# andrewcharlesjones/spatial-alignment

Measured on AMD Instinct MI355X. Metric: training steps/sec (ELBO fwd+bwd), 2-view N=10k M=200, 1/2/4/8 GPU, higher is better.
Workload: dtype f32 (fp64 warp layer, covariance whitening and M x M factorisations)

## Files before the change

include/gpsa_hip.h:

```cpp
#ifndef GPSA_HIP_H
#define GPSA_HIP_H

#ifdef __cplusplus
extern "C" {
#endif

enum {
  GPSA_F32 = 0,
  GPSA_F64 = 1,
  GPSA_F32_X64 = 2,
  GPSA_F32_OUT64 = 3,
  GPSA_F32_ACC64 = 4
};
enum { GPSA_K_RBF = 0, GPSA_K_MATERN12 = 1, GPSA_K_MATERN32 = 2 };
enum { GPSA_EINVAL = -1, GPSA_EWORKSPACE = -2, GPSA_EUNSUPPORTED = -3 };

int gpsa_version(void);
const char* gpsa_build_arch(void);
const char* gpsa_source_hash(void);

int gpsa_kmat(int dtype, int in_dtype, int kind, const void* Z, int M, const void* X, long long C,
              int D, const void* ls_u, const void* var_u, double jitter, void* K, void* stream);

long long gpsa_kmat_bwd_workspace(int dtype, int M, long long C, int D);
// ... 93 lines not shown
                                     long long workspace_bytes, void* stream);

long long gpsa_whiten_workspace(int M);
int gpsa_whiten_f64(const double* Kinv, int in_dtype, const void* Kuf, int M, long long C,
                    int alpha_dtype, void* alpha, double* q, void* workspace, long long workspace_bytes,
                    void* stream);

int gpsa_panel_mm(int dtype, int p_dtype, int transP, const void* P, const void* X, int M, long long C,
                  void* Y, void* colsq, void* workspace, long long workspace_bytes, void* stream);

int gpsa_col_axpy(int dtype, const void* Y, const void* X, const void* d, double s, int M,
                  long long C, void* out, void* stream);

int gpsa_data_sample_fwd(const float* meanT, const float* v, const double* q, const float* var_u,
                         const float* eps, long long C, int L, float* F, float* Sigma, void* stream);
int gpsa_data_sample_bwd(const float* dF, const float* eps, const float* Sigma, const float* var_u,
                         long long C, int L, float* g, float* dmeanT, float* qbar, int dvar_dtype, void* dvar_u,
                         void* workspace, long long workspace_bytes, void* stream);
int gpsa_warp_sample_fwd(const double* meanT, const double* v, const double* q, const float* var_u,
                         const float* X, const float* slopes, const float* intercept,
                         const float* eps, long long n, int D, int S, float* Gmean, float* Gs,
                         double* Gs64, int* bad, void* stream);
int gpsa_warp_sample_bwd(const float* dGmean, const float* dGs, const double* dGs64, const float* eps,
                         const float* var_u, const float* X, long long n, int D, int S, double* dmeanT, double* g,
                         double* qbar, float* dvar_u, float* dslopes, float* dintercept,
                         void* workspace, long long workspace_bytes, void* stream);

int gpsa_mean_resid_fwd(const float* Z, const float* slopes, const float* intercept,
                        const float* delta, int M, int D, double scale, float* mu_z, double* resid,
                        void* stream);
int gpsa_mean_resid_bwd(const double* dresid, const float* Z, const float* slopes, int M, int D,
                        double scale, float* ddelta, float* dZ, float* dslopes, float* dintercept,
                        void* stream);

int gpsa_loglik_fwd(const float* F, const float* Y, const float* noise_u, int S, long long N, int P,
                    double* out, void* workspace, long long workspace_bytes, void* stream);
int gpsa_loglik_bwd(const float* F, const float* Y, const float* noise_u, const double* gout, int S,
                    long long N, int P, float* dF, float* dnoise_u, void* workspace,
                    long long workspace_bytes, void* stream);

int gpsa_bdot(int dtype, const void* A, long long strideA, const void* B, long long strideB,
              long long n, int batch, void* out, void* workspace, long long workspace_bytes,
              void* stream);
int gpsa_add_diag(int dtype, void* A, int M, int batch, double s, void* stream);

int gpsa_mvn_kl_fwd(const double* Kinv, const double* logdetK, const double* Omega,
                    long long omega_stride, const double* logdetO, long long logdet_stride,
                    const double* Dm, const double* KD, int M, int L, double* kl, void* stream);
int gpsa_mvn_kl_bwd(const double* Kuu, const double* Kinv, const double* Omega, long long omega_stride,
                    const double* Oinv, long long oinv_stride, const double* Dm, const double* KD,
                    const double* g, int M, int L, double* dOmega, double* dDm, double* Sp,
                    void* stream);

int gpsa_mvn_kl_grouped_fwd(const double* mats, const double* inv, const double* logdet,
                            const int* om_idx, const int* pr_idx, const double* D, int M, int T,
                            double* kl, double* KD, void* stream);
int gpsa_mvn_kl_grouped_bwd(const double* mats, const double* inv, const int* om_idx,
                            const int* pr_list, const int* grp_off, const int* order, const double* D,
                            const double* KD, const double* g, int M, int T, int P, double* dOmega,
                            double* dD, double* S, void* stream);

int gpsa_elbo_fwd(const double* ll, int n_ll, const double* kl, int n_kl, double kl_scale, float* loss,
                  void* stream);
int gpsa_elbo_bwd(const float* gloss, int n_ll, int n_kl, double kl_scale, double* dll, double* dkl,
                  void* stream);

long long gpsa_kmeans_workspace(long long N, int D, int K);
int gpsa_kmeans_assign(const float* X, long long N, int D, const float* centres, int K, int* assign,
                       float* d2, void* stream);
int gpsa_kmeans_update(const float* X, const int* assign, long long N, int D, int K, float* centres,
                       int* counts, void* workspace, long long workspace_bytes, void* stream);


int gpsa_kmat_batched(int kind, const float* Z, long long strideZ, int M, const float* X, long long strideX,
                      long long C, int D, const float* ls_u, const float* var_u, int stride_par,
                      const long long* n_live, int batch, double jitter, double* K, long long strideK,
                      void* stream);
long long gpsa_kmat_bwd_batched_workspace(int M, long long C, int D, int batch);
int gpsa_kmat_bwd_batched(int kind, const float* Z, long long strideZ, int M, const float* X, long long strideX,
                          long long C, int D, const float* ls_u, const float* var_u, int stride_par,
                          const long long* n_live, int batch, const double* Kbar, long long strideK, int same,
                          double* dZ, long long stride_dZ, double* dparams, void* workspace,
                          long long workspace_bytes, void* stream);
int gpsa_kmat_bwd_x64(int kind, const float* Z, int M, const double* X, long long C, int D, const float* ls_u,
                      const float* var_u, const float* Kbar, double* dZ, double* dX, double* dparams,
                      void* workspace, long long workspace_bytes, void* stream);
int gpsa_kmat_bwd_x64_f64(int kind, const float* Z, int M, const double* X, long long C, int D, const float* ls_u,
                          const float* var_u, const double* Kbar, double* dZ, double* dX, double* dparams,
                          void* workspace, long long workspace_bytes, void* stream);
int gpsa_kmat_bwd_x64_f64_axpy(int kind, const float* Z, int M, const double* X, long long C, int D, const float* ls_u,
                               const float* var_u, const double* Kbar, const double* X2, const float* d, double s,
                               double* dZ, double* dX, double* dparams, void* workspace, long long workspace_bytes,
                               void* stream);
long long gpsa_exact_dkuu_workspace(int M, long long C);
int gpsa_exact_dkuu_f64(const double* G, const double* A, const float* d, int M, long long C, double* dK,
                        void* workspace, long long workspace_bytes, void* stream);
long long gpsa_longk_f64_workspace(int M, long long K, int nprob);
int gpsa_longk_f64(int nprob, const double* const* G, const double* const* B, const void* const* d, int d_dtype,
                   int M, long long K, long long ld, int sym, const double* alpha, const double* beta,
                   double* const* out, void* workspace, long long workspace_bytes, void* stream);
int gpsa_kmat_bwd_x64_axpy(int kind, const float* Z, int M, const double* X, long long C, int D, const float* ls_u,
                           const float* var_u, const float* Kbar, const float* X2, const float* d, double s,
                           double* dZ, double* dX, double* dparams, void* workspace, long long workspace_bytes,
                           void* stream);
int gpsa_whiten_f64_dual(const double* Kinv, const double* Kuf, int M, long long C, double* alpha64, float* alpha32,
                         double* q, void* workspace, long long workspace_bytes, void* stream);

int gpsa_whiten_gen_f64_dual(const double* Kinv, int kind, const float* Z, const double* X64, int D, const float* ls_u,
                             const float* var_u, int M, long long C, double* alpha64, float* alpha32, double* q,
                             void* workspace, long long workspace_bytes, void* stream);
int gpsa_whiten_axpy_f32(const double* Kinv, const float* X, int M, long long C, const float* X2, const float* d,
                         double s, float* out, void* workspace, long long workspace_bytes, void* stream);
int gpsa_whiten_batched_f64(const double* Kinv, long long strideKinv, const double* Kuf, int M, long long C,
                            long long strideX, double* alpha, double* q, int batch, void* workspace,
                            long long workspace_bytes, void* stream);
int gpsa_quadform_fwd_keep_batched_f64(const double* alpha, const double* Omega, int M, long long C, int L,
                                       double* v, double* W, const double* dcT, double* meanT, int batch,
                                       void* stream);
int gpsa_quadform_bwd_alpha_kept_batched_f64(const double* W, const double* g, int M, long long C, int L,
                                             const double* dcT, const double* dmeanT, double* dalpha,
                                             int batch, void* stream);
int gpsa_col_axpy_batched_f64(const double* Y, const double* X, const double* d, double s, int M, long long C,
                              double* out, int batch, void* stream);
long long gpsa_gram_batched_workspace(int M, long long C, int L, int batch);
int gpsa_gram_batched_f64(const double* alpha, const double* g, int M, long long C, int L, double* dOmega,
                          int batch, void* workspace, long long workspace_bytes, void* stream);
int gpsa_mvn_kl_grouped_bwd_acc(const double* mats, const double* inv, const int* om_idx,
                                const int* pr_list, const int* grp_off, const int* order, const double* D,
                                const double* KD, const double* g, int M, int T, int P, double* dOmega,
                                double* dD, double* S, int accumulate, void* stream);

#define GPSA_MAX_MODS 4

typedef struct gpsa_step_desc {
  int n_views, n_dims, n_mods, n_samples;
  int m_x, m_g;
  int kind_warp, kind_data;
  int n_latent[GPSA_MAX_MODS];
  int n_out[GPSA_MAX_MODS];
  int has_lmc[GPSA_MAX_MODS];
  long long n_rows[GPSA_MAX_MODS];
  int s_test;
  long long n_test[GPSA_MAX_MODS];
  int want_kl;
  const int* view_fixed;
  const long long* view_rows;
  long long keep_budget_bytes;
  int exact_inducing_grad;
  int kl_own_lo, kl_own_hi;
  int contraction;
} gpsa_step_desc;

typedef struct gpsa_step_params {
  const float* Xtilde;
  const float* delta_G;
  const float* Omega_sqt_G;
  const float* warp_ls;
  const float* warp_var;
  const float* slopes;
  const float* intercepts;
  const float* Gtilde;
  const float* data_ls;
  const float* data_var;
  const float* Omega_sqt_F[GPSA_MAX_MODS];
  const float* delta_F[GPSA_MAX_MODS];
  const float* W[GPSA_MAX_MODS];
} gpsa_step_params;

typedef struct gpsa_step_param_grads {
  float *Xtilde, *delta_G, *Omega_sqt_G, *warp_ls, *warp_var, *Gtilde, *data_ls, *data_var;
  float* Omega_sqt_F[GPSA_MAX_MODS];
  float* delta_F[GPSA_MAX_MODS];
  float* W[GPSA_MAX_MODS];
} gpsa_step_param_grads;

typedef struct gpsa_step_io {
  const float* X[GPSA_MAX_MODS];
  const float* eps_G;
  const float* eps_F[GPSA_MAX_MODS];
  const float* G_test[GPSA_MAX_MODS];
  const float* eps_F_test[GPSA_MAX_MODS];
  float* G_means[GPSA_MAX_MODS];
  float* G_samples[GPSA_MAX_MODS];
  float* F_latent[GPSA_MAX_MODS];
  float* F_obs[GPSA_MAX_MODS];
  float* F_latent_test[GPSA_MAX_MODS];
  float* F_obs_test[GPSA_MAX_MODS];
  float* mu_z;
  double* kl;
  int* flag;
  int keep_products;
  int reuse_mm;
  int fuse_elbo;
  const float* Y[GPSA_MAX_MODS];
  const float* noise_u[GPSA_MAX_MODS];
  double* ll_part[GPSA_MAX_MODS];
  float* F_fused_T[GPSA_MAX_MODS];
  double* bwd_acc;
  int bwd_acc_mode;
  void* f_event;
  const float* loss_src;
  float* loss_dst;
  int skip_missing;
} gpsa_step_io;

typedef struct gpsa_step_out_grads {
  const float* dG_means[GPSA_MAX_MODS];
  const float* dG_samples[GPSA_MAX_MODS];
  const float* dF_latent[GPSA_MAX_MODS];
  const float* dF_obs[GPSA_MAX_MODS];
  const float* dF_latent_test[GPSA_MAX_MODS];
  const float* dF_obs_test[GPSA_MAX_MODS];
  const double* dkl;
// ... 139 lines not shown
```

spatial_alignment_amd/_lib.py:

```python
import ctypes as C
import os

_HERE = os.path.dirname(os.path.abspath(__file__))
LIB_PATH = os.path.join(_HERE, "libgpsa_hip.so")

_vp, _i, _ll, _d = C.c_void_p, C.c_int, C.c_longlong, C.c_double

SIGNATURES = {
    "gpsa_version": (_i, []),
    "gpsa_build_arch": (C.c_char_p, []),
    "gpsa_source_hash": (C.c_char_p, []),
    "gpsa_kmat": (_i, [_i, _i, _i, _vp, _i, _vp, _ll, _i, _vp, _vp, _d, _vp, _vp]),
    "gpsa_kmat_bwd_workspace": (_ll, [_i, _i, _ll, _i]),
    "gpsa_kmat_bwd": (_i, [_i, _i, _i, _vp, _i, _vp, _ll, _i, _vp, _vp, _vp, _i, _vp, _vp, _vp, _vp, _ll, _vp]),
    "gpsa_gemm_workspace": (_ll, [_i, _i, _i, _i, _i]),
    "gpsa_gemm": (_i, [_i, _i, _i, _i, _i, _ll, _d, _vp, _ll, _ll, _vp, _ll, _ll, _d, _vp, _ll, _ll,
                       _i, _i, _vp, _ll, _vp]),
    "gpsa_omega_fwd": (_i, [_vp, _i, _i, _d, _vp, _vp]),
    "gpsa_omega_bwd": (_i, [_vp, _vp, _i, _i, _i, _vp, _vp]),
    "gpsa_omega_fwd2": (_i, [_vp, _i, _vp, _vp, _i, _vp, _i, _d, _vp]),
    "gpsa_omega_bwd2": (_i, [_vp, _vp, _vp, _i, _vp, _vp, _vp, _i, _i, _i, _vp]),
    "gpsa_chol_f64": (_i, [_vp, _i, _i, _vp, _vp, _vp]),
    "gpsa_tri_inv_f64": (_i, [_vp, _vp, _i, _i, _vp]),
    "gpsa_chol_inv_f64": (_i, [_vp, _vp, _i, _i, _vp, _vp, _vp]),
# ... 15 lines not shown
    "gpsa_quadform_bwd_omega_delta_x3": (_i, [_i, _vp, _vp, _vp, _i, _ll, _i, _vp, _vp, _d, _vp, _ll, _vp]),
    "gpsa_whiten_workspace": (_ll, [_i]),
    "gpsa_whiten_f64": (_i, [_vp, _i, _vp, _i, _ll, _i, _vp, _vp, _vp, _ll, _vp]),
    "gpsa_panel_mm": (_i, [_i, _i, _i, _vp, _vp, _i, _ll, _vp, _vp, _vp, _ll, _vp]),
    "gpsa_col_axpy": (_i, [_i, _vp, _vp, _vp, _d, _i, _ll, _vp, _vp]),
    "gpsa_data_sample_fwd": (_i, [_vp, _vp, _vp, _vp, _vp, _ll, _i, _vp, _vp, _vp]),
    "gpsa_data_sample_bwd": (_i, [_vp, _vp, _vp, _vp, _ll, _i, _vp, _vp, _vp, _i, _vp, _vp, _ll, _vp]),
    "gpsa_warp_sample_fwd": (_i, [_vp, _vp, _vp, _vp, _vp, _vp, _vp, _vp, _ll, _i, _i, _vp, _vp, _vp, _vp, _vp]),
    "gpsa_warp_sample_bwd": (_i, [_vp, _vp, _vp, _vp, _vp, _vp, _ll, _i, _i, _vp, _vp, _vp, _vp, _vp, _vp, _vp,
                                  _ll, _vp]),
    "gpsa_mean_resid_fwd": (_i, [_vp, _vp, _vp, _vp, _i, _i, _d, _vp, _vp, _vp]),
    "gpsa_mean_resid_bwd": (_i, [_vp, _vp, _vp, _i, _i, _d, _vp, _vp, _vp, _vp, _vp]),
    "gpsa_loglik_fwd": (_i, [_vp, _vp, _vp, _i, _ll, _i, _vp, _vp, _ll, _vp]),
    "gpsa_loglik_bwd": (_i, [_vp, _vp, _vp, _vp, _i, _ll, _i, _vp, _vp, _vp, _ll, _vp]),
    "gpsa_bdot": (_i, [_i, _vp, _ll, _vp, _ll, _ll, _i, _vp, _vp, _ll, _vp]),
    "gpsa_add_diag": (_i, [_i, _vp, _i, _i, _d, _vp]),
    "gpsa_mvn_kl_fwd": (_i, [_vp, _vp, _vp, _ll, _vp, _ll, _vp, _vp, _i, _i, _vp, _vp]),
    "gpsa_mvn_kl_bwd": (_i, [_vp, _vp, _vp, _ll, _vp, _ll, _vp, _vp, _vp, _i, _i, _vp, _vp, _vp, _vp]),
    "gpsa_mvn_kl_grouped_fwd": (_i, [_vp, _vp, _vp, _vp, _vp, _vp, _i, _i, _vp, _vp, _vp]),
    "gpsa_mvn_kl_grouped_bwd": (_i, [_vp, _vp, _vp, _vp, _vp, _vp, _vp, _vp, _vp, _i, _i, _i, _vp, _vp, _vp,
                                     _vp]),
    "gpsa_elbo_fwd": (_i, [_vp, _i, _vp, _i, _d, _vp, _vp]),
    "gpsa_elbo_bwd": (_i, [_vp, _i, _i, _d, _vp, _vp, _vp]),
    "gpsa_kmeans_workspace": (_ll, [_ll, _i, _i]),
    "gpsa_kmeans_assign": (_i, [_vp, _ll, _i, _vp, _i, _vp, _vp, _vp]),
    "gpsa_kmeans_update": (_i, [_vp, _vp, _ll, _i, _i, _vp, _vp, _vp, _ll, _vp]),
}

MAX_MODS = 4


class StepDesc(C.Structure):
    _fields_ = [
        ("n_views", _i), ("n_dims", _i), ("n_mods", _i), ("n_samples", _i),
        ("m_x", _i), ("m_g", _i), ("kind_warp", _i), ("kind_data", _i),
        ("n_latent", _i * MAX_MODS), ("n_out", _i * MAX_MODS), ("has_lmc", _i * MAX_MODS),
        ("n_rows", _ll * MAX_MODS), ("s_test", _i), ("n_test", _ll * MAX_MODS), ("want_kl", _i),
        ("view_fixed", C.POINTER(_i)), ("view_rows", C.POINTER(_ll)), ("keep_budget_bytes", _ll),
        ("exact_inducing_grad", _i), ("kl_own_lo", _i), ("kl_own_hi", _i), ("contraction", _i),
    ]


class StepParams(C.Structure):
    _fields_ = [
        ("Xtilde", _vp), ("delta_G", _vp), ("Omega_sqt_G", _vp), ("warp_ls", _vp), ("warp_var", _vp),
        ("slopes", _vp), ("intercepts", _vp), ("Gtilde", _vp), ("data_ls", _vp), ("data_var", _vp),
        ("Omega_sqt_F", _vp * MAX_MODS), ("delta_F", _vp * MAX_MODS), ("W", _vp * MAX_MODS),
    ]


class StepParamGrads(C.Structure):
    _fields_ = [
        ("Xtilde", _vp), ("delta_G", _vp), ("Omega_sqt_G", _vp), ("warp_ls", _vp), ("warp_var", _vp),
        ("Gtilde", _vp), ("data_ls", _vp), ("data_var", _vp),
        ("Omega_sqt_F", _vp * MAX_MODS), ("delta_F", _vp * MAX_MODS), ("W", _vp * MAX_MODS),
    ]


class StepIO(C.Structure):
    _fields_ = [
        ("X", _vp * MAX_MODS), ("eps_G", _vp), ("eps_F", _vp * MAX_MODS), ("G_test", _vp * MAX_MODS),
        ("eps_F_test", _vp * MAX_MODS), ("G_means", _vp * MAX_MODS), ("G_samples", _vp * MAX_MODS),
        ("F_latent", _vp * MAX_MODS), ("F_obs", _vp * MAX_MODS), ("F_latent_test", _vp * MAX_MODS),
        ("F_obs_test", _vp * MAX_MODS), ("mu_z", _vp), ("kl", _vp), ("flag", _vp), ("keep_products", _i),
        ("reuse_mm", _i), ("fuse_elbo", _i), ("Y", _vp * MAX_MODS), ("noise_u", _vp * MAX_MODS),
        ("ll_part", _vp * MAX_MODS), ("F_fused_T", _vp * MAX_MODS), ("bwd_acc", _vp), ("bwd_acc_mode", _i),
        ("f_event", _vp), ("loss_src", _vp), ("loss_dst", _vp), ("skip_missing", _i),
    ]


class StepOutGrads(C.Structure):
    _fields_ = [
        ("dG_means", _vp * MAX_MODS), ("dG_samples", _vp * MAX_MODS), ("dF_latent", _vp * MAX_MODS),
        ("dF_obs", _vp * MAX_MODS), ("dF_latent_test", _vp * MAX_MODS), ("dF_obs_test", _vp * MAX_MODS),
        ("dkl", _vp), ("gloss", _vp),
    ]


_pp = C.POINTER(_vp)

SIGNATURES.update({
    "gpsa_kmat_batched": (_i, [_i, _vp, _ll, _i, _vp, _ll, _ll, _i, _vp, _vp, _i, C.POINTER(_ll), _i, _d, _vp, _ll, _vp]),
    "gpsa_kmat_bwd_batched_workspace": (_ll, [_i, _ll, _i, _i]),
    "gpsa_kmat_bwd_batched": (_i, [_i, _vp, _ll, _i, _vp, _ll, _ll, _i, _vp, _vp, _i, C.POINTER(_ll), _i, _vp, _ll, _i,
                                   _vp, _ll, _vp, _vp, _ll, _vp]),
    "gpsa_kmat_bwd_x64": (_i, [_i, _vp, _i, _vp, _ll, _i, _vp, _vp, _vp, _vp, _vp, _vp, _vp, _ll, _vp]),
    "gpsa_kmat_bwd_x64_f64": (_i, [_i, _vp, _i, _vp, _ll, _i, _vp, _vp, _vp, _vp, _vp, _vp, _vp, _ll, _vp]),
    "gpsa_kmat_bwd_x64_f64_axpy": (_i, [_i, _vp, _i, _vp, _ll, _i, _vp, _vp, _vp, _vp, _vp, _d, _vp, _vp, _vp, _vp, _ll,
                                        _vp]),
    "gpsa_exact_dkuu_workspace": (_ll, [_i, _ll]),
    "gpsa_exact_dkuu_f64": (_i, [_vp, _vp, _vp, _i, _ll, _vp, _vp, _ll, _vp]),
    "gpsa_longk_f64_workspace": (_ll, [_i, _ll, _i]),
    "gpsa_longk_f64": (_i, [_i, _vp, _vp, _vp, _i, _i, _ll, _ll, _i, _vp, _vp, _vp, _vp, _ll, _vp]),
    "gpsa_kmat_bwd_x64_axpy": (_i, [_i, _vp, _i, _vp, _ll, _i, _vp, _vp, _vp, _vp, _vp, _d, _vp, _vp, _vp, _vp, _ll,
                                    _vp]),
    "gpsa_thin_update_f32": (_i, [_vp, _i, _i, _vp, _ll, _vp, _vp]),
    "gpsa_whiten_f64_dual": (_i, [_vp, _vp, _i, _ll, _vp, _vp, _vp, _vp, _ll, _vp]),
    "gpsa_whiten_gen_f64_dual": (_i, [_vp, _i, _vp, _vp, _i, _vp, _vp, _i, _ll, _vp, _vp, _vp, _vp, _ll, _vp]),
    "gpsa_whiten_axpy_f32": (_i, [_vp, _vp, _i, _ll, _vp, _vp, _d, _vp, _vp, _ll, _vp]),
    "gpsa_whiten_batched_f64": (_i, [_vp, _ll, _vp, _i, _ll, _ll, _vp, _vp, _i, _vp, _ll, _vp]),
    "gpsa_quadform_fwd_keep_batched_f64": (_i, [_vp, _vp, _i, _ll, _i, _vp, _vp, _vp, _vp, _i, _vp]),
    "gpsa_quadform_bwd_alpha_kept_batched_f64": (_i, [_vp, _vp, _i, _ll, _i, _vp, _vp, _vp, _i, _vp]),
    "gpsa_col_axpy_batched_f64": (_i, [_vp, _vp, _vp, _d, _i, _ll, _vp, _i, _vp]),
    "gpsa_gram_batched_workspace": (_ll, [_i, _ll, _i, _i]),
    "gpsa_gram_batched_f64": (_i, [_vp, _vp, _i, _ll, _i, _vp, _i, _vp, _ll, _vp]),
    "gpsa_mvn_kl_grouped_bwd_acc": (_i, [_vp, _vp, _vp, _vp, _vp, _vp, _vp, _vp, _vp, _i, _i, _i, _vp, _vp, _vp, _i,
                                         _vp]),
    "gpsa_step_create": (_vp, [C.POINTER(StepDesc)]),
    "gpsa_step_describe": (_i, [C.POINTER(StepDesc), C.POINTER(_ll)]),
    "gpsa_step_destroy": (None, [_vp]),
    "gpsa_step_saved_bytes": (_ll, [_vp]),
    "gpsa_step_saved_bytes_nokeep": (_ll, [_vp]),
    "gpsa_quadform_keep_f32_workspace": (_ll, [_i, _i]),
    "gpsa_quadform_fwd_keep_f32": (_i, [_i, _vp, _vp, _i, _ll, _i, _vp, _vp, _vp, _ll, _vp]),
    "gpsa_quadform_keep_f32_bytes": (_ll, [_i, _ll, _i]),
    "gpsa_quadform_bwd_alpha_kept_f32": (_i, [_vp, _vp, _i, _ll, _i, _vp, _vp, _vp, _vp]),
    "gpsa_lmc_loglik_workspace": (_ll, [_ll, _i, _i, _i]),
    "gpsa_lmc_loglik_fused_f32": (_i, [_vp, _vp, _vp, _vp, _i, _ll, _i, _i, _vp, _i, _vp, _vp, _vp, _ll, _vp]),
    "gpsa_quadform_elbo_parts": (_i, []),
    "gpsa_quadform_elbo_f32_workspace": (_ll, [_i, _ll, _i]),
    "gpsa_quadform_elbo_f32": (_i, [_i, _vp, _vp, _i, _ll, _i, _vp, _vp, _vp, _vp, _vp, _ll, _i, _vp, _vp, _vp, _vp, _vp,
                                    _vp, _vp, _ll, _vp]),
    "gpsa_quadform_elbo_takes_delta": (_i, [_i]),
    "gpsa_quadform_elbo_x3_f32_workspace": (_ll, [_i, _ll, _i]),
    "gpsa_quadform_elbo_x3_f32": (_i, [_i, _vp, _vp, _i, _ll, _i, _vp, _vp, _vp, _vp, _vp, _ll, _i, _vp, _vp, _vp, _vp,
                                       _vp, _vp, _vp, _ll, _vp]),
    "gpsa_quadform_elbo_delta_x3_f32": (_i, [_i, _vp, _vp, _i, _ll, _i, _vp, _vp, _vp, _vp, _vp, _ll, _i, _vp, _vp, _vp,
                                             _vp, _vp, _vp, _vp, _ll, _vp]),
    "gpsa_quadform_elbo_delta_f32": (_i, [_i, _vp, _vp, _i, _ll, _i, _vp, _vp, _vp, _vp, _vp, _ll, _i, _vp, _vp, _vp, _vp,
                                          _vp, _vp, _vp, _ll, _vp]),
    "gpsa_step_scratch_bytes": (_ll, [_vp]),
    "gpsa_step_bwd_acc_bytes": (_ll, [_vp]),
    "gpsa_step_n_kl": (_i, [_vp]),
    "gpsa_step_n_factorised": (_i, [_vp]),
    "gpsa_step_eps_g_numel": (_ll, [_vp]),
    "gpsa_step_batch_layout": (_i, [_vp, C.POINTER(_ll)]),
    "gpsa_step_graph": (_i, [_vp, _i, C.POINTER(_ll)]),
    "gpsa_step_early_backwards": (_ll, [_vp]),
    "gpsa_stream_capture_id": (C.c_ulonglong, [_vp]),
    "gpsa_step_timing": (_i, [_vp, _i]),
    "gpsa_step_timing_read": (_i, [_vp, _vp, _i]),
    "gpsa_step_forward": (_i, [_vp, C.POINTER(StepParams), C.POINTER(StepIO), _vp, _vp, _i, _vp]),
    "gpsa_step_backward": (_i, [_vp, C.POINTER(StepParams), C.POINTER(StepIO), C.POINTER(StepOutGrads), _vp, _vp,
                                C.POINTER(StepParamGrads), _vp]),
    "gpsa_elbo_loss_fwd": (_i, [_i, _pp, _pp, _pp, C.POINTER(_i), C.POINTER(_ll), C.POINTER(_i), _vp, _i, _d, _vp,
                                _vp, _vp, _ll, _vp]),
    "gpsa_elbo_loss_bwd": (_i, [_i, _pp, _pp, _pp, C.POINTER(_i), C.POINTER(_ll), C.POINTER(_i), _vp, _i, _d, _pp, _pp,
                                _vp, _i, _vp, _vp, _ll, _vp]),
    "gpsa_elbo_loss_fused_fwd": (_i, [_i, _pp, _pp, _pp, C.POINTER(_i), C.POINTER(_ll), C.POINTER(_i), _pp, _i, _vp, _i,
                                      _d, _vp, _vp, _vp, _ll, _vp]),
    "gpsa_elbo_loss_fused_bwd": (_i, [_i, _pp, _pp, _pp, C.POINTER(_i), C.POINTER(_ll), C.POINTER(_i), _pp, _i, _vp, _i,
                                      _d, _pp, _pp, _vp, _i, _vp, _vp, _ll, _vp]),
    "gpsa_elbo_fused_post": (_i, [_vp, _vp, _vp, _i, _ll, _i, _vp, _vp, _i, _vp, _vp, _ll, _vp]),
    "gpsa_step_fused": (_i, [_vp, _i]),
    "gpsa_step_contraction": (_i, [_vp, _i]),
    "gpsa_adam_step": (_i, [_i, _pp, _pp, _pp, _pp, C.POINTER(_ll), _d, _d, _d, _d, _vp, _vp]),
    "gpsa_row_sample_gather": (_i, [_i, C.POINTER(_i), C.POINTER(_ll), C.POINTER(_ll), C.c_ulonglong, _vp, _pp,
                                    C.POINTER(_i), _pp, C.POINTER(_i), _pp, _pp, _pp, _vp]),
    "gpsa_elbo_loss_weighted_fwd": (_i, [_i, _pp, _pp, _pp, C.POINTER(_i), C.POINTER(_ll), C.POINTER(_i),
                                         C.POINTER(_i), _pp, _pp, _vp, _i, _d, _vp, _vp, _vp, _ll, _vp]),
    "gpsa_elbo_loss_weighted_bwd": (_i, [_i, _pp, _pp, _pp, C.POINTER(_i), C.POINTER(_ll), C.POINTER(_i),
                                         C.POINTER(_i), _pp, _pp, _vp, _i, _d, _pp, _pp, _vp, _i, _vp, _vp, _ll, _vp]),
    "gpsa_quadform_elbo_skip_f32": (_i, [_i, _vp, _vp, _i, _ll, _i, _vp, _vp, _vp, _vp, _vp, _ll, _i, _vp, _vp, _vp, _vp,
                                         _vp, _vp, _vp, _ll, _vp]),
    "gpsa_quadform_elbo_delta_skip_f32": (_i, [_i, _vp, _vp, _i, _ll, _i, _vp, _vp, _vp, _vp, _vp, _ll, _i, _vp, _vp, _vp,
                                               _vp, _vp, _vp, _vp, _ll, _vp]),
    "gpsa_count_observed_workspace": (_ll, []),
    "gpsa_count_observed": (_i, [_i, _pp, C.POINTER(_ll), C.POINTER(_i), C.POINTER(_i), _pp, _pp, _vp, _ll, _vp]),
    "gpsa_elbo_loss_skip_fwd": (_i, [_i, _pp, _pp, _pp, C.POINTER(_i), C.POINTER(_ll), C.POINTER(_i), _pp, _i,
                                     C.POINTER(_i), _pp, _pp, _pp, _vp, _i, _d, _vp, _vp, _vp, _ll, _vp]),
    "gpsa_elbo_loss_skip_bwd": (_i, [_i, _pp, _pp, _pp, C.POINTER(_i), C.POINTER(_ll), C.POINTER(_i), _pp, _i,
                                     C.POINTER(_i), _pp, _pp, _pp, _vp, _i, _d, _pp, _pp, _vp, _i, _vp, _vp, _ll, _vp]),
    "gpsa_lmc_loglik_fused_skip_f32": (_i, [_vp, _vp, _vp, _vp, _i, _ll, _i, _i, _vp, _i, _vp, _vp, _vp, _ll, _vp]),
    "gpsa_predict_moments_f32": (_i, [_vp, _vp, _vp, _vp, _ll, _i, _i, _i, _vp, _vp, _i, _vp, _vp, _vp, _vp, _vp, _vp,
                                      _vp]),
    "gpsa_predict_counts_f32": (_i, [_vp, _vp, _vp, _vp, _ll, _i, _i, _i, _vp, _vp, _vp, _vp, _vp, _vp, _vp]),
    "gpsa_lgamma_sum_workspace": (_ll, []),
    "gpsa_lgamma_sum": (_i, [_i, _pp, C.POINTER(_ll), C.POINTER(_i), C.POINTER(_i), _pp, _i, _pp, _vp, _ll, _vp]),
    "gpsa_elbo_loss_pois_fwd": (_i, [_i, _pp, _pp, _pp, C.POINTER(_i), C.POINTER(_ll), C.POINTER(_i), _pp, _i,
                                     C.POINTER(_i), _pp, _pp, _pp, C.POINTER(_i), _pp, _pp, _i, _vp, _i, _d, _vp, _vp,
                                     _vp, _ll, _vp]),
    "gpsa_elbo_loss_pois_bwd": (_i, [_i, _pp, _pp, _pp, C.POINTER(_i), C.POINTER(_ll), C.POINTER(_i), _pp, _i,
                                     C.POINTER(_i), _pp, _pp, _pp, C.POINTER(_i), _pp, _pp, _i, _vp, _i, _d, _pp, _pp,
                                     _vp, _i, _vp, _vp, _ll, _vp]),
    "gpsa_quadform_elbo_pois_f32": (_i, [_i, _vp, _vp, _i, _ll, _i, _vp, _vp, _vp, _vp, _vp, _ll, _i, _vp, _vp, _vp, _vp,
                                         _vp, _vp, _vp, _i, _vp, _ll, _vp]),
    "gpsa_quadform_elbo_delta_pois_f32": (_i, [_i, _vp, _vp, _i, _ll, _i, _vp, _vp, _vp, _vp, _vp, _ll, _i, _vp, _vp, _vp,
                                               _vp, _vp, _vp, _vp, _i, _vp, _ll, _vp]),
    "gpsa_lmc_loglik_fused_pois_f32": (_i, [_vp, _vp, _vp, _vp, _i, _i, _ll, _i, _i, _vp, _i, _vp, _vp, _vp, _ll, _vp]),
    "gpsa_step_likelihood": (_i, [_vp, _i, _i, _vp]),
# ... 73 lines not shown
```

spatial_alignment_amd/csrc/internal.hpp:

```cpp
#pragma once
#include "common.hpp"

namespace gpsa {

template <typename T>
int gemm_launch(int transA, int transB, int m, int n, long long k, double alpha, const T* A, long long lda,
                long long sA, const T* B, long long ldb, long long sB, double beta, T* C, long long ldc,
                long long sC, int batch, int splitk, void* ws, long long ws_bytes, hipStream_t st);
enum { GEMM_TRI_NONE = 0, GEMM_TRI_UPPER_A = 1, GEMM_TRI_LOWER_C = 2, GEMM_TRI_LTL = 3 };
template <typename T>
int gemm_launch_tri(int transA, int transB, int m, int n, long long k, double alpha, const T* A, long long lda,
                    long long sA, const T* B, long long ldb, long long sB, double beta, T* C, long long ldc,
                    long long sC, int batch, int splitk, void* ws, long long ws_bytes, hipStream_t st, int tri);
template <typename TIA, typename TIB, typename TO>
int gemm64_launch(int transA, int transB, int m, int n, long long k, double alpha, const TIA* A, long long lda,
                  long long sA, const TIB* B, long long ldb, long long sB, double beta, TO* C, long long ldc,
                  long long sC, int batch, int splitk, void* ws, long long ws_bytes, hipStream_t st);

int omega_fwd_dma_launch(const float* A0, int n0, double* O0, const float* A1, int n1, double* O1, int M, double jitter,
                         hipStream_t st);

int omega_bwd_dma_launch(const double* G0, const float* A0, float* D0, int n0, const double* G1, const float* A1,
                         float* D1, int n1, int M, hipStream_t st);

int mvn_kl_grouped_fwd_slices(int M);
int mvn_kl_grouped_fwd_copy(const double* mats, const double* inv, const double* logdet, const int* om_idx,
                            const int* pr_idx, const double* D, int M, int T, double* kl, double* KD,
                            double* kl_copy, double* part, int* cnt, hipStream_t st);

int lmc_mfma_launch(const float* F, const float* W, const float* Y, const float* noise_u, int S, long long N, int L,
                    int P, double* zpart, int nparts, float* dF, float* dWpart, int G, hipStream_t st);
int lmc_mfma_skip_launch(const float* F, const float* W, const float* Y, const float* noise_u, int S, long long N, int L,
                         int P, double* zpart, int nparts, float* dF, float* dWpart, int G, hipStream_t st);

constexpr int LOSS_MAX_VIEWS = 64;
struct ViewRows {
  long long off[LOSS_MAX_VIEWS + 1];
};
static inline bool views_ok(int V, const long long* off, long long N) {
  if (V < 1 || V > LOSS_MAX_VIEWS || off == nullptr || off[0] != 0 || off[V] != N) return false;
  for (int v = 0; v < V; ++v)
    if (off[v + 1] < off[v]) return false;
  return true;
}
static inline ViewRows view_rows(long long N, int V, const long long* off) {
  ViewRows vr;
  if (off != nullptr) {
    for (int v = 0; v <= V; ++v) vr.off[v] = off[v];
  } else {
    vr.off[0] = 0;
    vr.off[1] = N;
  }
  return vr;
}

int pois_loglik_launch(bool bwd, const float* F, const float* Y, const float* log_offset, int S, long long N, int P,
                       const ViewRows& vr, int V, int nb, const double* w, const float* gloss, int skip, float* dF,
                       double* part, hipStream_t st);
int lmc_mfma_pois_launch(const float* F, const float* W, const float* Y, const float* log_offset, int skip, int S,
                         long long N, int L, int P, double* zpart, int nparts, float* dF, float* dWpart, int G,
                         hipStream_t st);

bool proj64_ok(int MB, long long C, int batch);
template <typename TI>
int proj64_launch(int MB, const double* Apk, const TI* X, int M, long long C, double* alpha, float* out32, double* q,
                  int batch, long long sX, hipStream_t st, bool q_zeroed);
int zero_fill_async(void* ptr, size_t bytes, hipStream_t st);
int copy_async(void* dst, const void* src, size_t bytes, hipStream_t st);
int elbo_fused_post_ticket(float* g_ext, float* dmeanT, float* abar, int M, long long C, int L, const float* gloss,
                           const float* var_u, double* dvar_u, double* part, int* tick, hipStream_t st);
int proj64_gen_launch(int MB, const double* Apk, int kind, const float* Z, const double* X64, int D, const float* ls_u,
                      const float* var_u, int M, long long C, double* alpha, float* out32, double* q, hipStream_t st,
                      bool q_zeroed);

}
```

spatial_alignment_amd/csrc/kl.hip:

```cpp
#include "common.hpp"

namespace gpsa {

__global__ void __launch_bounds__(1024)
mvn_kl_fwd_kernel(const double* __restrict__ Kinv, const double* __restrict__ logdetK,
                  const double* __restrict__ Omega, long long omega_stride,
                  const double* __restrict__ logdetO, long long logdet_stride,
                  const double* __restrict__ Dm, const double* __restrict__ KD, int M, int L,
                  double* __restrict__ kl) {
  __shared__ double red[16];
  const int l = blockIdx.x;
  const double* Om = Omega + (long long)l * omega_stride;
  double acc = 0.0;
  for (int e = threadIdx.x; e < M * M; e += 1024) acc += Kinv[e] * Om[e];
  for (int m = threadIdx.x; m < M; m += 1024) acc += KD[(long long)m * L + l] * Dm[(long long)m * L + l];
  const double t = block_sum(acc, red);
  if (threadIdx.x == 0)
    kl[l] = 0.5 * (logdetK[0] - logdetO[(long long)l * logdet_stride] + t - (double)M);
}

__global__ void __launch_bounds__(256)
mvn_kl_bwd_kernel(const double* __restrict__ Kuu, const double* __restrict__ Kinv,
                  const double* __restrict__ Omega, long long omega_stride,
                  const double* __restrict__ Oinv, long long oinv_stride,
// ... 23 lines not shown
                          const int* __restrict__ pr_idx, const double* __restrict__ D, int M,
                          double* __restrict__ kl, double* __restrict__ KD, double* __restrict__ kl_copy,
                          double* part, int* cnt) {
  __shared__ double red[16];
  const int t = blockIdx.x, lane = threadIdx.x & 63, w = threadIdx.x >> 6;
  const int q = blockIdx.y, NS = gridDim.y;
  const int p = pr_idx[t], o = om_idx[t];
  if (p < 0) {
    if (q != 0) return;
    if (threadIdx.x == 0) {
      kl[t] = 0.0;
      if (kl_copy != nullptr) kl_copy[t] = 0.0;
    }
    for (int m = threadIdx.x; m < M; m += 1024) KD[(long long)t * M + m] = 0.0;
    return;
  }
  const double* Ki = inv + (long long)p * M * M;
  const double* Om = mats + (long long)o * M * M;
  const double* d = D + (long long)t * M;
  double acc = 0.0;
  for (int i0 = w + 64 * q; i0 < M; i0 += 64 * NS) {
    double tr[4] = {0.0, 0.0, 0.0, 0.0}, kd[4] = {0.0, 0.0, 0.0, 0.0};
    for (int j0 = 0; j0 < M; j0 += 256) {
      double kv[4][4], ov[4][4], dv[4];
#pragma unroll
      for (int q = 0; q < 4; ++q) {
        const int j = j0 + lane + 64 * q;
        dv[q] = j < M ? d[j < M ? j : M - 1] : 0.0;
#pragma unroll
        for (int r = 0; r < 4; ++r) {
          const int i = i0 + 16 * r;
          const long long e = (long long)(i < M ? i : M - 1) * M + (j < M ? j : M - 1);
          kv[r][q] = Ki[e];
          ov[r][q] = Om[e];
        }
      }
#pragma unroll
      for (int r = 0; r < 4; ++r)
#pragma unroll
        for (int q = 0; q < 4; ++q) {
          const bool ok = i0 + 16 * r < M && j0 + lane + 64 * q < M;
          const double k = ok ? kv[r][q] : 0.0;
          tr[r] += k * ov[r][q];
          kd[r] += k * dv[q];
        }
    }
#pragma unroll
    for (int r = 0; r < 4; ++r) {
      const int i = i0 + 16 * r;
      if (i < M) {
        const double s = wave_sum(kd[r]);
        if (lane == 0) {
          KD[(long long)t * M + i] = s;
          acc += s * d[i];
        }
        acc += tr[r];
      }
    }
  }
  double tot = block_sum(acc, red);
  if (threadIdx.x == 0) {
    if (NS > 1) {
      part[(long long)t * NS + q] = tot;
      __threadfence();
      if (atomicAdd(&cnt[t], 1) != NS - 1) return;
      __threadfence();
      tot = 0.0;
      for (int i = 0; i < NS; ++i) tot += __hip_atomic_load(&part[(long long)t * NS + i], __ATOMIC_RELAXED, __HIP_MEMORY_SCOPE_AGENT);
      cnt[t] = 0;
    }
    const double v = 0.5 * (logdet[p] - logdet[o] + tot - (double)M);
    kl[t] = v;
    if (kl_copy != nullptr) kl_copy[t] = v;
  }
}

__global__ void __launch_bounds__(256)
mvn_kl_grouped_bwd_kernel(const double* __restrict__ mats, const double* __restrict__ inv,
                          const int* __restrict__ om_idx,
                          const int* __restrict__ pr_list, const int* __restrict__ grp_off,
                          const int* __restrict__ order, const double* __restrict__ D,
                          const double* __restrict__ KD, const double* __restrict__ g, int M, int T, int P,
                          double* __restrict__ dOmega, double* __restrict__ dD, double* __restrict__ S,
                          int accumulate) {
  const long long mm = (long long)M * M, e = blockIdx.x * 256LL + threadIdx.x;
  const int pg = blockIdx.y;
  const int t0 = grp_off[pg], t1 = grp_off[pg + 1];
  if (pg == P) {
    if (blockIdx.x == 0)
      for (int q = t0; q < t1; ++q)
        for (int m = threadIdx.x; m < M; m += 256) dD[(long long)order[q] * M + m] = 0.0;
    if (!accumulate && e < mm)
      for (int q = t0; q < t1; ++q) dOmega[(long long)order[q] * mm + e] = 0.0;
    return;
  }
  const int p = pr_list[pg];
  if (blockIdx.x == 0)
    for (int q = t0; q < t1; ++q) {
      const int t = order[q];
      for (int m = threadIdx.x; m < M; m += 256) dD[(long long)t * M + m] = g[t] * KD[(long long)t * M + m];
    }
  if (e >= mm) return;
  const int i = (int)(e / M), j = (int)(e % M);
  const double kinv = inv[(long long)p * mm + e];
  double s0 = 0.0, s1 = 0.0, gs = 0.0;
  for (int q = t0; q < t1; q += 8) {
    double ga[8], om[8], oi[8], di[8], dj[8], old[8];
    int tt[8];
#pragma unroll
    for (int u = 0; u < 8; ++u) {
      const bool on = q + u < t1;
      const int ta = order[on ? q + u : t0];
      tt[u] = on ? ta : -1;
      ga[u] = on ? g[ta] : 0.0;
      const long long mo = (long long)om_idx[ta] * mm + e;
      om[u] = mats[mo];
      oi[u] = inv[mo];
      di[u] = D[(long long)ta * M + i];
      dj[u] = D[(long long)ta * M + j];
      old[u] = (accumulate && on) ? dOmega[(long long)ta * mm + e] : 0.0;
    }
#pragma unroll
    for (int u = 0; u < 8; ++u)
      if (tt[u] >= 0) dOmega[(long long)tt[u] * mm + e] = old[u] + 0.5 * ga[u] * (kinv - oi[u]);
#pragma unroll
    for (int u = 0; u < 8; u += 2) {
      gs += ga[u] + ga[u + 1];
      s0 += ga[u] * (om[u] + di[u] * dj[u]);
      s1 += ga[u + 1] * (om[u + 1] + di[u + 1] * dj[u + 1]);
    }
  }
  S[(long long)pg * mm + e] = gs * mats[(long long)p * mm + e] - (s0 + s1);
}

int mvn_kl_grouped_fwd_slices(int M) { return M > 64 ? (M + 63) / 64 < 8 ? (M + 63) / 64 : 8 : 1; }
int mvn_kl_grouped_fwd_copy(const double* mats, const double* inv, const double* logdet, const int* om_idx,
                            const int* pr_idx, const double* D, int M, int T, double* kl, double* KD,
                            double* kl_copy, double* part, int* cnt, hipStream_t st) {
  if (M < 1 || T < 1) return GPSA_EINVAL;
  const int ns = (part != nullptr && cnt != nullptr) ? mvn_kl_grouped_fwd_slices(M) : 1;
  mvn_kl_grouped_fwd_kernel<<<dim3((unsigned)T, (unsigned)ns), 1024, 0, st>>>(mats, inv, logdet, om_idx, pr_idx, D, M, kl,
                                                                             KD, kl_copy, part, cnt);
  GPSA_LAUNCH_CHECK();
  return 0;
}

}

extern "C" {

int gpsa_mvn_kl_grouped_fwd(const double* mats, const double* inv, const double* logdet,
                            const int* om_idx, const int* pr_idx, const double* D, int M, int T,
                            double* kl, double* KD, void* stream) {
  if (M < 1 || T < 1) return GPSA_EINVAL;
  gpsa::mvn_kl_grouped_fwd_kernel<<<T, 1024, 0, as_stream(stream)>>>(mats, inv, logdet, om_idx, pr_idx, D,
                                                                     M, kl, KD, nullptr, nullptr, nullptr);
  GPSA_LAUNCH_CHECK();
  return 0;
}

int gpsa_mvn_kl_grouped_bwd_acc(const double* mats, const double* inv, const int* om_idx,
                                const int* pr_list, const int* grp_off, const int* order, const double* D,
                                const double* KD, const double* g, int M, int T, int P, double* dOmega,
                                double* dD, double* S, int accumulate, void* stream) {
  if (M < 1 || T < 1 || P < 1) return GPSA_EINVAL;
  dim3 grid((unsigned)cdiv((long long)M * M, 256), (unsigned)(P + 1));
  gpsa::mvn_kl_grouped_bwd_kernel<<<grid, 256, 0, as_stream(stream)>>>(
      mats, inv, om_idx, pr_list, grp_off, order, D, KD, g, M, T, P, dOmega, dD, S, accumulate);
  GPSA_LAUNCH_CHECK();
  return 0;
}

int gpsa_mvn_kl_grouped_bwd(const double* mats, const double* inv, const int* om_idx,
                            const int* pr_list, const int* grp_off, const int* order, const double* D,
                            const double* KD, const double* g, int M, int T, int P, double* dOmega,
                            double* dD, double* S, void* stream) {
  return gpsa_mvn_kl_grouped_bwd_acc(mats, inv, om_idx, pr_list, grp_off, order, D, KD, g, M, T, P, dOmega,
                                     dD, S, 0, stream);
}

int gpsa_mvn_kl_fwd(const double* Kinv, const double* logdetK, const double* Omega,
                    long long omega_stride, const double* logdetO, long long logdet_stride,
                    const double* Dm, const double* KD, int M, int L, double* kl, void* stream) {
  if (M < 1 || L < 1) return GPSA_EINVAL;
  gpsa::mvn_kl_fwd_kernel<<<L, 1024, 0, as_stream(stream)>>>(Kinv, logdetK, Omega, omega_stride, logdetO,
                                                             logdet_stride, Dm, KD, M, L, kl);
  GPSA_LAUNCH_CHECK();
  return 0;
}

int gpsa_mvn_kl_bwd(const double* Kuu, const double* Kinv, const double* Omega, long long omega_stride,
                    const double* Oinv, long long oinv_stride, const double* Dm, const double* KD,
                    const double* g, int M, int L, double* dOmega, double* dDm, double* Sp,
                    void* stream) {
  if (M < 1 || L < 1) return GPSA_EINVAL;
  const unsigned nb = (unsigned)cdiv((long long)M * M, 256);
  gpsa::mvn_kl_bwd_kernel<<<nb, 256, 0, as_stream(stream)>>>(Kuu, Kinv, Omega, omega_stride, Oinv,
                                                             oinv_stride, Dm, KD, g, M, L, dOmega, dDm, Sp);
  GPSA_LAUNCH_CHECK();
  return 0;
}

}
```

spatial_alignment_amd/csrc/kmat.hip:

```cpp
#include "common.hpp"
#include "kmat_cov.hpp"

namespace gpsa {

constexpr int KM_ROWS = 16;

constexpr int KM_MAXB = 16;
struct KmatBatch {
  long long sZ, sX, sK;
  int sP, ragged;
  long long n[KM_MAXB];
  const void* axX;
  const float* axd;
  float axs;
};
static inline KmatBatch kmat_single() {
  KmatBatch kb;
  kb.sZ = kb.sX = kb.sK = 0;
  kb.sP = kb.ragged = 0;
  kb.axX = nullptr;
  kb.axd = nullptr;
  kb.axs = 0.f;
  for (int i = 0; i < KM_MAXB; ++i) kb.n[i] = 0;
  return kb;
}

template <typename TI, typename TX, typename T, int KIND>
__global__ void __launch_bounds__(256)
kmat_fwd_kernel(const TI* __restrict__ Z, int M, const TX* __restrict__ X, long long C, int D,
                const TI* __restrict__ ls_u, const TI* __restrict__ var_u, T jitter,
                T* __restrict__ K, KmatBatch kb) {
  __shared__ T Zs[KM_ROWS][MAXD];
  const int b = blockIdx.z;
  Z += b * kb.sZ;
  X += b * kb.sX;
  K += b * kb.sK;
  ls_u += b * kb.sP;
  var_u += b * kb.sP;
  const long long live = kb.ragged ? kb.n[b] : C;
  const int m0 = blockIdx.y * KM_ROWS;
  if (threadIdx.x < KM_ROWS * MAXD) {
    int r = threadIdx.x / MAXD, d = threadIdx.x % MAXD;
    Zs[r][d] = (m0 + r < M && d < D) ? (T)Z[(long long)(m0 + r) * D + d] : T(0);
  }
  __syncthreads();
  const long long c = blockIdx.x * 256LL + threadIdx.x;
  if (c >= C) return;
  const int mend = min(KM_ROWS, M - m0);
  if (c >= live) {
    for (int r = 0; r < mend; ++r) K[(long long)(m0 + r) * C + c] = T(0);
    return;
  }
  const T ell = t_exp<T>((T)ls_u[0]), inv_ell = T(1) / ell, var = t_exp<T>((T)var_u[0]);
  T x[MAXD];
#pragma unroll
  for (int d = 0; d < MAXD; ++d) x[d] = (d < D) ? (T)X[c * D + d] : T(0);
  for (int r = 0; r < mend; ++r) {
    T k, cd, pl;
    cov_eval<T, KIND>(Zs[r], x, D, ell, inv_ell, var, k, cd, pl);
    if ((long long)(m0 + r) == c) k += jitter;
    K[(long long)(m0 + r) * C + c] = k;
  }
}

constexpr int KB_MCHUNK = 32;
constexpr int KB_MCHUNK_SMALL = 8;
static inline int kb_rows(int M, long long C) {
  return (cdiv(C, 256) * cdiv(M, KB_MCHUNK) < 1024) ? KB_MCHUNK_SMALL : KB_MCHUNK;
}
constexpr int KB_MAXBX = 1024;
constexpr int KB_D2_ROWS = 16;
static inline int kmat_bwd_d2_rows() { return KB_D2_ROWS; }
static inline bool kmat_bwd_d2(int M, long long Ctot, int D) {
  (void)M;
  (void)Ctot;
  return D == 2;
}

template <typename TI, typename T, int KIND, int MCH, typename TK = T, typename TX = TI>
__global__ void __launch_bounds__(256)
kmat_bwd_kernel(const TI* __restrict__ Z, int M, const TX* __restrict__ X, long long C, int D,
                const TI* __restrict__ ls_u, const TI* __restrict__ var_u,
                const TK* __restrict__ Kbar, T* __restrict__ zpart, T* __restrict__ xpart,
                T* __restrict__ spart, KmatBatch bt) {
  {
    const long long b = blockIdx.z;
    Z += b * bt.sZ;
    X += b * bt.sX;
    Kbar += b * bt.sK;
    ls_u += b * bt.sP;
    var_u += b * bt.sP;
    zpart += b * (long long)gridDim.x * M * D;
    if (xpart != nullptr) xpart += b * (long long)gridDim.y * C * D;
    spart += b * (long long)gridDim.x * gridDim.y * 2;
  }
  const long long nlive = bt.ragged ? bt.n[blockIdx.z] : C;
  __shared__ T Zs[MCH][MAXD];
  __shared__ T acc[4][MCH][MAXD];
  __shared__ T red[4];
  const int lane = threadIdx.x & 63, w = threadIdx.x >> 6;
  const int m0 = blockIdx.y * MCH;
  const int mc = min(MCH, M - m0);
  const T ell = t_exp<T>((T)ls_u[0]), inv_ell = T(1) / ell, var = t_exp<T>((T)var_u[0]);
  if (threadIdx.x < MCH * MAXD) {
    const int r = threadIdx.x / MAXD, d = threadIdx.x % MAXD;
    Zs[r][d] = (r < mc && d < D) ? (T)Z[(long long)(m0 + r) * D + d] : T(0);
  }
  for (int i = threadIdx.x; i < 4 * MCH * MAXD; i += 256) (&acc[0][0][0])[i] = T(0);
  __syncthreads();
  T s_ls = T(0), s_var = T(0);
  const long long ncb = (C + 255) / 256;
  for (long long cb = blockIdx.x; cb < ncb; cb += gridDim.x) {
    const long long c = cb * 256 + threadIdx.x;
    const bool live = c < nlive;
    T x[MAXD], dx[MAXD];
#pragma unroll
    for (int d = 0; d < MAXD; ++d) {
      x[d] = (live && d < D) ? (T)X[c * D + d] : T(0);
      dx[d] = T(0);
    }
    const T axc = (bt.axX != nullptr && live) ? (T)bt.axs * (T)bt.axd[c] : T(0);
    for (int r = 0; r < mc; ++r) {
      T k, cd, pl;
      cov_eval<T, KIND>(Zs[r], x, D, ell, inv_ell, var, k, cd, pl);
      T kb = live ? (T)Kbar[(long long)(m0 + r) * C + c] : T(0);
      if (bt.axX != nullptr && live)
        kb += axc * (T)reinterpret_cast<const TK*>(bt.axX)[(long long)(m0 + r) * C + c];
      s_ls += kb * pl;
      s_var += kb * k;
      T wgt = kb * cd;
#pragma unroll
      for (int d = 0; d < MAXD; ++d)
        if (d < D) {
          T t = wgt * (Zs[r][d] - x[d]);
          dx[d] -= t;
          T tz = wave_sum(t);
          if (lane == 0) acc[w][r][d] += tz;
        }
    }
    if (xpart != nullptr && c < C) {
      T* xr = xpart + (long long)blockIdx.y * C * D;
      for (int d = 0; d < D; ++d) xr[c * D + d] = dx[d];
    }
  }
  __syncthreads();
  T* zrow = zpart + (long long)blockIdx.x * M * D;
  for (int i = threadIdx.x; i < mc * D; i += 256) {
    const int r = i / D, d = i % D;
    zrow[(long long)(m0 + r) * D + d] = acc[0][r][d] + acc[1][r][d] + acc[2][r][d] + acc[3][r][d];
  }
  T* sp = spart + ((long long)blockIdx.x * gridDim.y + blockIdx.y) * 2;
  T a = block_sum(s_ls, red);
  if (threadIdx.x == 0) sp[0] = a;
  T b2 = block_sum(s_var, red);
  if (threadIdx.x == 0) sp[1] = b2;
}

template <typename TI, typename T, int KIND, int MCH, typename TK = T, typename TX = TI>
__global__ void __launch_bounds__(256, 2)
kmat_bwd_d2_kernel(const TI* __restrict__ Z, int M, int rows, const TX* __restrict__ X, long long C,
                   const TI* __restrict__ ls_u, const TI* __restrict__ var_u,
                   const TK* __restrict__ Kbar, T* __restrict__ zpart, T* __restrict__ xpart,
                   T* __restrict__ spart, KmatBatch bt) {
  constexpr int D = 2;
  static_assert(MCH % 8 == 0, "the closing reduction takes 8 rows at a time");
  {
    const long long b = blockIdx.z;
    Z += b * bt.sZ;
    X += b * bt.sX;
    Kbar += b * bt.sK;
    ls_u += b * bt.sP;
    var_u += b * bt.sP;
    zpart += b * (long long)gridDim.x * M * D;
    if (xpart != nullptr) xpart += b * (long long)gridDim.y * C * D;
    spart += b * (long long)gridDim.x * gridDim.y * 2;
  }
  const long long nlive = bt.ragged ? bt.n[blockIdx.z] : C;
  constexpr int RSTR = 256 + 16;
  __shared__ T Zs[MCH][MAXD];
  __shared__ T rbuf[16 * RSTR];
  __shared__ T red[4];
  const int m0 = blockIdx.y * rows;
  const int mc = min(rows, M - m0);
  const T ell = t_exp<T>((T)ls_u[0]), inv_ell = T(1) / ell, var = t_exp<T>((T)var_u[0]);
  if (threadIdx.x < MCH * MAXD) {
    const int r = threadIdx.x / MAXD, d = threadIdx.x % MAXD;
    Zs[r][d] = (r < mc && d < D) ? (T)Z[(long long)(m0 + r) * D + d] : T(0);
  }
  __syncthreads();
  T tz[MCH][D];
#pragma unroll
  for (int r = 0; r < MCH; ++r) tz[r][0] = tz[r][1] = T(0);
  T s_ls = T(0), s_var = T(0);
  const long long ncb = (C + 255) / 256;
  struct Col {
    long long c;
    bool live;
    T x0, x1, axc;
  };
  const bool two = bt.axX != nullptr;
  const TK* __restrict__ axp = reinterpret_cast<const TK*>(bt.axX);
  auto load = [&](long long cb, TK(&kraw)[MCH], TK(&araw)[MCH], Col& q) {
    q.c = cb * 256 + threadIdx.x;
    q.live = q.c < nlive;
    q.x0 = q.x1 = q.axc = T(0);
    const long long cc = q.live ? q.c : 0;
    if (q.live) {
      q.x0 = (T)X[q.c * D];
      q.x1 = (T)X[q.c * D + 1];
    }
    if (two) {
      if (q.live) q.axc = (T)bt.axs * (T)bt.axd[q.c];
#pragma unroll
      for (int r = 0; r < MCH; ++r) {
        const long long o = (long long)min(m0 + r, M - 1) * C + cc;
        kraw[r] = Kbar[o];
        araw[r] = axp[o];
      }
    } else {
#pragma unroll
      for (int r = 0; r < MCH; ++r) {
        kraw[r] = Kbar[(long long)min(m0 + r, M - 1) * C + cc];
        araw[r] = TK(0);
      }
    }
  };
  auto compute = [&](const TK(&kraw)[MCH], const TK(&araw)[MCH], const Col& q) {
    const T x[MAXD] = {q.x0, q.x1, T(0), T(0)};
    T dx0 = T(0), dx1 = T(0);
    int zo = 0;
    asm volatile("" : "+v"(zo));
    const T(*Zr)[MAXD] = Zs + zo;
#pragma unroll
    for (int r = 0; r < MCH; ++r) {
      T k, cd, pl;
      cov_eval<T, KIND>(Zr[r], x, D, ell, inv_ell, var, k, cd, pl);
      const T kb = (q.live && r < mc) ? (T)kraw[r] + q.axc * (T)araw[r] : T(0);
      s_ls += kb * pl;
      s_var += kb * k;
      const T wgt = kb * cd;
      const T t0 = wgt * (Zr[r][0] - x[0]), t1 = wgt * (Zr[r][1] - x[1]);
      dx0 -= t0;
      dx1 -= t1;
      tz[r][0] += t0;
      tz[r][1] += t1;
      if ((r & 3) == 3) __builtin_amdgcn_sched_barrier(0);
    }
    if (xpart != nullptr && q.c < C) {
      T* xr = xpart + (long long)blockIdx.y * C * D;
      xr[q.c * D] = dx0;
      xr[q.c * D + 1] = dx1;
    }
  };
  for (long long cb = blockIdx.x; cb < ncb; cb += gridDim.x) {
    TK k0[MCH];
    TK a0[MCH];
    Col q0;
    load(cb, k0, a0, q0);
    __builtin_amdgcn_sched_barrier(0);
    compute(k0, a0, q0);
  }
  T* zrow = zpart + (long long)blockIdx.x * M * D;
#pragma unroll
  for (int r0 = 0; r0 < MCH; r0 += 8) {
    __syncthreads();
#pragma unroll
    for (int q = 0; q < 8; ++q) {
      rbuf[(2 * q) * RSTR + threadIdx.x] = tz[r0 + q][0];
      rbuf[(2 * q + 1) * RSTR + threadIdx.x] = tz[r0 + q][1];
    }
    __syncthreads();
    const int v = threadIdx.x >> 4, sub = threadIdx.x & 15;
    T a = T(0);
#pragma unroll
    for (int i = 0; i < 16; ++i) a += rbuf[v * RSTR + sub + 16 * i];
    a += dpp_move<0xB1>(a);
    a += dpp_move<0x4E>(a);
    a += dpp_move<0x141>(a);
    a += dpp_move<0x140>(a);
    const int r = r0 + (v >> 1);
    if (sub == 0 && r < mc) zrow[(long long)(m0 + r) * D + (v & 1)] = a;
  }
  T* sp = spart + ((long long)blockIdx.x * gridDim.y + blockIdx.y) * 2;
  T a = block_sum(s_ls, red);
  if (threadIdx.x == 0) sp[0] = a;
  T b2 = block_sum(s_var, red);
  if (threadIdx.x == 0) sp[1] = b2;
}

template <typename T, typename TO>
__global__ void __launch_bounds__(256)
kmat_bwd_finish_kernel(const T* __restrict__ zpart, long long nbx, long long nz,
                       const T* __restrict__ xpart, long long nby, long long nx,
                       const T* __restrict__ spart, long long ns, int same, TO* __restrict__ dZ,
                       TO* __restrict__ dX, TO* __restrict__ dparams, long long sdZ, long long sdX) {
  {
    const long long b = blockIdx.y;
    zpart += b * nbx * nz;
    if (xpart != nullptr) xpart += b * nby * nx;
    spart += b * ns * 2;
    dZ += b * sdZ;
    if (dX != nullptr) dX += b * sdX;
    dparams += b * 2;
  }
  __shared__ double red[256];
  const long long zb = (nz + 15) / 16, xb = (nx + 63) / 64;
  const T* part;
  long long rows, stride, n, col;
  int ng, grp, sub;
  TO* dst;
  long long blk = blockIdx.x;
  bool fold = false;
  if (blk < zb) {
    ng = 16; grp = threadIdx.x >> 4; sub = threadIdx.x & 15;
    part = zpart; rows = nbx; stride = nz; n = nz; col = blk * 16 + sub; dst = dZ; fold = same != 0;
  } else if (blk < zb + xb) {
    blk -= zb;
    if (xpart == nullptr || dX == nullptr || same) return;
    ng = 4; grp = threadIdx.x >> 6; sub = threadIdx.x & 63;
    part = xpart; rows = nby; stride = nx; n = nx; col = blk * 64 + sub; dst = dX;
  } else {
    ng = 16; grp = threadIdx.x >> 4; sub = threadIdx.x & 15;
    part = spart; rows = ns; stride = 2; n = 2; col = sub; dst = dparams;
  }
  double a0 = 0.0, a1 = 0.0, a2 = 0.0, a3 = 0.0;
  if (col < n) {
    long long r = grp;
    for (; r + 3 * ng < rows; r += 4 * ng) {
      a0 += (double)part[r * stride + col];
      a1 += (double)part[(r + ng) * stride + col];
      a2 += (double)part[(r + 2 * ng) * stride + col];
      a3 += (double)part[(r + 3 * ng) * stride + col];
    }
    for (; r < rows; r += ng) a0 += (double)part[r * stride + col];
    if (fold)
      for (long long q = grp; q < nby; q += ng) a1 += (double)xpart[q * nx + col];
  }
  const int width = 256 / ng;
  red[grp * width + sub] = (a0 + a1) + (a2 + a3);
  __syncthreads();
  if (grp == 0 && col < n) {
    double t = 0.0;
    for (int q = 0; q < ng; ++q) t += red[q * width + sub];
    dst[col] = (TO)t;
  }
}

template <typename TI, typename TX, typename T>
int kmat_launch(int kind, const TI* Z, int M, const TX* X, long long C, int D, const TI* ls_u,
                const TI* var_u, double jitter, T* K, hipStream_t st, int batch = 1,
                KmatBatch kb = kmat_single()) {
  if (batch < 1 || batch > KM_MAXB) return GPSA_EINVAL;
  dim3 grid((unsigned)cdiv(C, 256), (unsigned)cdiv(M, KM_ROWS), (unsigned)batch);
  switch (kind) {
    case GPSA_K_RBF:
      kmat_fwd_kernel<TI, TX, T, GPSA_K_RBF><<<grid, 256, 0, st>>>(Z, M, X, C, D, ls_u, var_u, (T)jitter, K, kb);
      break;
    case GPSA_K_MATERN12:
      kmat_fwd_kernel<TI, TX, T, GPSA_K_MATERN12><<<grid, 256, 0, st>>>(Z, M, X, C, D, ls_u, var_u, (T)jitter, K, kb);
      break;
    case GPSA_K_MATERN32:
      kmat_fwd_kernel<TI, TX, T, GPSA_K_MATERN32><<<grid, 256, 0, st>>>(Z, M, X, C, D, ls_u, var_u, (T)jitter, K, kb);
      break;
    default:
      return GPSA_EINVAL;
  }
  GPSA_LAUNCH_CHECK();
  return 0;
}

template <typename TI, typename T, typename TO = TI, typename TK = T, typename TX = TI>
int kmat_bwd_launch(int kind, const TI* Z, int M, const TX* X, long long C, int D, const TI* ls_u,
                    const TI* var_u, const TK* Kbar, TO* dZ, TO* dX, TO* dparams, int same, void* ws,
                    long long ws_bytes, hipStream_t st, int batch = 1, KmatBatch kb = kmat_single(),
                    long long sdZ = 0, long long sdX = 0) {
  if (batch < 1 || batch > KM_MAXB) return GPSA_EINVAL;
  const int mch = kb_rows(M, C * batch);
  const long long ncb = cdiv(C, 256), nby = cdiv(M, mch);
  long long nbx = ncb < KB_MAXBX ? ncb : KB_MAXBX;
  const long long nz = (long long)M * D, nx = C * D;
  const long long need = (nbx * nz + nby * nx + nbx * nby * 2) * (long long)sizeof(T) * batch;
  const bool d2 = kmat_bwd_d2(M, C * batch, D);
  if (!d2 && ws_bytes < need) return GPSA_EWORKSPACE;
  T* zpart = reinterpret_cast<T*>(ws);
  T* xpart = zpart + nbx * nz * batch;
  T* spart = xpart + nby * nx * batch;
  T* xp = (dX || same) ? xpart : nullptr;
  if (d2) {
    const int mr = kmat_bwd_d2_rows();
    const long long nby2 = cdiv(M, mr);
    const long long slots = 2LL * num_cus();
    long long per = 1;
    while (per < ncb && cdiv(ncb, per) * nby2 * batch > slots) ++per;
    nbx = cdiv(ncb, per);
    const int rows = (int)cdiv(M, nby2);
    if ((nbx * nz + nby2 * nx + nbx * nby2 * 2) * (long long)sizeof(T) * batch > ws_bytes) return GPSA_EWORKSPACE;
    xpart = zpart + nbx * nz * batch;
    spart = xpart + nby2 * nx * batch;
    xp = (dX || same) ? xpart : nullptr;
    dim3 grid((unsigned)nbx, (unsigned)nby2, (unsigned)batch);
#define GPSA_KB_CASE(KIND)                                                                                     \
  kmat_bwd_d2_kernel<TI, T, KIND, KB_D2_ROWS, TK, TX><<<grid, 256, 0, st>>>(Z, M, rows, X, C, ls_u, var_u, Kbar, \
                                                                            zpart, xp, spart, kb);
    switch (kind) {
      case GPSA_K_RBF: GPSA_KB_CASE(GPSA_K_RBF) break;
      case GPSA_K_MATERN12: GPSA_KB_CASE(GPSA_K_MATERN12) break;
      case GPSA_K_MATERN32: GPSA_KB_CASE(GPSA_K_MATERN32) break;
      default:
        return GPSA_EINVAL;
    }
#undef GPSA_KB_CASE
    GPSA_LAUNCH_CHECK();
    const bool fold2 = same != 0;
    if (fold2 && (nx != nz)) return GPSA_EINVAL;
    dim3 fgrid2((unsigned)(cdiv(nz, 16) + cdiv(nx, 64) + 1), (unsigned)batch);
    kmat_bwd_finish_kernel<T, TO><<<fgrid2, 256, 0, st>>>(zpart, nbx, nz, xp, nby2, nx, spart, nbx * nby2,
                                                          fold2 ? 1 : 0, dZ, dX, dparams, sdZ, sdX);
    GPSA_LAUNCH_CHECK();
    return 0;
  }
  dim3 grid((unsigned)nbx, (unsigned)nby, (unsigned)batch);
#define GPSA_KB_CASE(KIND)                                                                          \
  if (mch == KB_MCHUNK)                                                                             \
    kmat_bwd_kernel<TI, T, KIND, KB_MCHUNK, TK, TX><<<grid, 256, 0, st>>>(Z, M, X, C, D, ls_u, var_u, \
                                                                      Kbar, zpart, xp, spart, kb);  \
  else                                                                                              \
    kmat_bwd_kernel<TI, T, KIND, KB_MCHUNK_SMALL, TK, TX><<<grid, 256, 0, st>>>(Z, M, X, C, D, ls_u, \
                                                                            var_u, Kbar, zpart, xp, \
                                                                            spart, kb);
  switch (kind) {
    case GPSA_K_RBF: GPSA_KB_CASE(GPSA_K_RBF) break;
    case GPSA_K_MATERN12: GPSA_KB_CASE(GPSA_K_MATERN12) break;
    case GPSA_K_MATERN32: GPSA_KB_CASE(GPSA_K_MATERN32) break;
    default:
      return GPSA_EINVAL;
  }
#undef GPSA_KB_CASE
  GPSA_LAUNCH_CHECK();
  const bool fold = same != 0;
  if (fold && (nx != nz)) return GPSA_EINVAL;
  dim3 fgrid((unsigned)(cdiv(nz, 16) + cdiv(nx, 64) + 1), (unsigned)batch);
  kmat_bwd_finish_kernel<T, TO><<<fgrid, 256, 0, st>>>(zpart, nbx, nz, xp, nby, nx, spart, nbx * nby,
                                                       fold ? 1 : 0, dZ, dX, dparams, sdZ, sdX);
  GPSA_LAUNCH_CHECK();
  return 0;
}

}

extern "C" {

int gpsa_kmat(int dtype, int in_dtype, int kind, const void* Z, int M, const void* X, long long C,
              int D, const void* ls_u, const void* var_u, double jitter, void* K, void* stream) {
  if (D < 1 || D > gpsa::MAXD || M < 1 || C < 1) return GPSA_EINVAL;
  hipStream_t st = as_stream(stream);
  if (dtype == GPSA_F32 && in_dtype == GPSA_F32)
    return gpsa::kmat_launch<float, float, float>(kind, (const float*)Z, M, (const float*)X, C, D,
                                           (const float*)ls_u, (const float*)var_u, jitter, (float*)K, st);
  if (dtype == GPSA_F64 && in_dtype == GPSA_F64)
    return gpsa::kmat_launch<double, double, double>(kind, (const double*)Z, M, (const double*)X, C, D,
                                             (const double*)ls_u, (const double*)var_u, jitter, (double*)K, st);
  if (dtype == GPSA_F64 && in_dtype == GPSA_F32)
    return gpsa::kmat_launch<float, float, double>(kind, (const float*)Z, M, (const float*)X, C, D,
                                                   (const float*)ls_u, (const float*)var_u, jitter, (double*)K, st);
  if (dtype == GPSA_F64 && in_dtype == GPSA_F32_X64)
    return gpsa::kmat_launch<float, double, double>(kind, (const float*)Z, M, (const double*)X, C, D,
                                                    (const float*)ls_u, (const float*)var_u, jitter, (double*)K, st);
  return GPSA_EINVAL;
}

long long gpsa_kmat_bwd_workspace(int dtype, int M, long long C, int D) {
  const long long nbx = cdiv(C, 256);
  long long nby = cdiv(M, gpsa::kb_rows(M, C));
  if (gpsa::kmat_bwd_d2(M, C, D)) nby = cdiv(M, gpsa::kmat_bwd_d2_rows());
  return (nbx * M * D + nby * C * D + nbx * nby * 2) * (dtype == GPSA_F64 ? 8 : 4);
}

int gpsa_kmat_bwd(int dtype, int in_dtype, int kind, const void* Z, int M, const void* X, long long C,
                  int D, const void* ls_u, const void* var_u, const void* Kbar, int same, void* dZ,
                  void* dX, void* dparams, void* workspace, long long workspace_bytes, void* stream) {
  if (D < 1 || D > gpsa::MAXD || M < 1 || C < 1) return GPSA_EINVAL;
  hipStream_t st = as_stream(stream);
  if (dtype == GPSA_F32 && in_dtype == GPSA_F32)
    return gpsa::kmat_bwd_launch<float, float>(kind, (const float*)Z, M, (const float*)X, C, D,
                                               (const float*)ls_u, (const float*)var_u, (const float*)Kbar,
                                               (float*)dZ, (float*)dX, (float*)dparams, same, workspace,
                                               workspace_bytes, st);
  if (dtype == GPSA_F64 && in_dtype == GPSA_F64)
    return gpsa::kmat_bwd_launch<double, double>(kind, (const double*)Z, M, (const double*)X, C, D,
                                                 (const double*)ls_u, (const double*)var_u,
                                                 (const double*)Kbar, (double*)dZ, (double*)dX,
                                                 (double*)dparams, same, workspace, workspace_bytes, st);
  if (dtype == GPSA_F64 && in_dtype == GPSA_F32)
    return gpsa::kmat_bwd_launch<float, double>(kind, (const float*)Z, M, (const float*)X, C, D,
                                                (const float*)ls_u, (const float*)var_u,
                                                (const double*)Kbar, (float*)dZ, (float*)dX,
                                                (float*)dparams, same, workspace, workspace_bytes, st);
  if (dtype == GPSA_F64 && in_dtype == GPSA_F32_OUT64)
    return gpsa::kmat_bwd_launch<float, double, double>(kind, (const float*)Z, M, (const float*)X, C, D,
                                                        (const float*)ls_u, (const float*)var_u,
                                                        (const double*)Kbar, (double*)dZ, (double*)dX,
                                                        (double*)dparams, same, workspace, workspace_bytes, st);
  if (dtype == GPSA_F64 && in_dtype == GPSA_F32_ACC64)
    return gpsa::kmat_bwd_launch<float, double, double, float>(
        kind, (const float*)Z, M, (const float*)X, C, D, (const float*)ls_u, (const float*)var_u,
        (const float*)Kbar, (double*)dZ, (double*)dX, (double*)dparams, same, workspace, workspace_bytes, st);
  return GPSA_EINVAL;
}

static gpsa::KmatBatch make_batch(long long sZ, long long sX, long long sK, int sP, const long long* n_live,
                                  int batch) {
  gpsa::KmatBatch kb = gpsa::kmat_single();
  kb.sZ = sZ;
  kb.sX = sX;
  kb.sK = sK;
  kb.sP = sP;
  kb.ragged = n_live != nullptr;
  for (int i = 0; i < batch && i < gpsa::KM_MAXB; ++i) kb.n[i] = n_live ? n_live[i] : 0;
  return kb;
}

int gpsa_kmat_batched(int kind, const float* Z, long long strideZ, int M, const float* X, long long strideX,
                      long long C, int D, const float* ls_u, const float* var_u, int stride_par,
                      const long long* n_live, int batch, double jitter, double* K, long long strideK,
                      void* stream) {
  if (D < 1 || D > gpsa::MAXD || M < 1 || C < 1 || batch < 1 || batch > gpsa::KM_MAXB) return GPSA_EINVAL;
  return gpsa::kmat_launch<float, float, double>(kind, Z, M, X, C, D, ls_u, var_u, jitter, K, as_stream(stream),
                                                 batch, make_batch(strideZ, strideX, strideK, stride_par, n_live, batch));
}

long long gpsa_kmat_bwd_batched_workspace(int M, long long C, int D, int batch) {
  const int mch = gpsa::kb_rows(M, C * batch);
  const long long ncb = cdiv(C, 256), nbx = ncb < gpsa::KB_MAXBX ? ncb : gpsa::KB_MAXBX;
  long long nby = cdiv(M, mch);
  if (gpsa::kmat_bwd_d2(M, C * batch, D)) nby = cdiv(M, gpsa::kmat_bwd_d2_rows());
  return (nbx * M * D + nby * C * D + nbx * nby * 2) * 8LL * batch;
}

int gpsa_kmat_bwd_batched(int kind, const float* Z, long long strideZ, int M, const float* X, long long strideX,
                          long long C, int D, const float* ls_u, const float* var_u, int stride_par,
                          const long long* n_live, int batch, const double* Kbar, long long strideK, int same,
                          double* dZ, long long stride_dZ, double* dparams, void* workspace,
                          long long workspace_bytes, void* stream) {
  if (D < 1 || D > gpsa::MAXD || M < 1 || C < 1 || batch < 1 || batch > gpsa::KM_MAXB) return GPSA_EINVAL;
  return gpsa::kmat_bwd_launch<float, double, double, double, float>(
      kind, Z, M, X, C, D, ls_u, var_u, Kbar, dZ, (double*)nullptr, dparams, same, workspace, workspace_bytes,
      as_stream(stream), batch, make_batch(strideZ, strideX, strideK, stride_par, n_live, batch), stride_dZ, 0);
}

int gpsa_kmat_bwd_x64(int kind, const float* Z, int M, const double* X, long long C, int D, const float* ls_u,
                      const float* var_u, const float* Kbar, double* dZ, double* dX, double* dparams,
                      void* workspace, long long workspace_bytes, void* stream) {
  return gpsa_kmat_bwd_x64_axpy(kind, Z, M, X, C, D, ls_u, var_u, Kbar, nullptr, nullptr, 0.0, dZ, dX, dparams,
                                workspace, workspace_bytes, stream);
}

int gpsa_kmat_bwd_x64_f64(int kind, const float* Z, int M, const double* X, long long C, int D, const float* ls_u,
                          const float* var_u, const double* Kbar, double* dZ, double* dX, double* dparams,
                          void* workspace, long long workspace_bytes, void* stream) {
  return gpsa_kmat_bwd_x64_f64_axpy(kind, Z, M, X, C, D, ls_u, var_u, Kbar, nullptr, nullptr, 0.0, dZ, dX, dparams,
                                    workspace, workspace_bytes, stream);
}

int gpsa_kmat_bwd_x64_f64_axpy(int kind, const float* Z, int M, const double* X, long long C, int D, const float* ls_u,
                               const float* var_u, const double* Kbar, const double* X2, const float* d, double s,
                               double* dZ, double* dX, double* dparams, void* workspace, long long workspace_bytes,
                               void* stream) {
  if (D < 1 || D > gpsa::MAXD || M < 1 || C < 1) return GPSA_EINVAL;
  if ((X2 == nullptr) != (d == nullptr)) return GPSA_EINVAL;
  gpsa::KmatBatch kb = gpsa::kmat_single();
  kb.axX = X2;
  kb.axd = d;
  kb.axs = (float)s;
  return gpsa::kmat_bwd_launch<float, double, double, double, double>(
      kind, Z, M, X, C, D, ls_u, var_u, Kbar, dZ, dX, dparams, 0, workspace, workspace_bytes, as_stream(stream), 1, kb);
}

int gpsa_kmat_bwd_x64_axpy(int kind, const float* Z, int M, const double* X, long long C, int D, const float* ls_u,
                           const float* var_u, const float* Kbar, const float* X2, const float* d, double s,
                           double* dZ, double* dX, double* dparams, void* workspace, long long workspace_bytes,
                           void* stream) {
  if (D < 1 || D > gpsa::MAXD || M < 1 || C < 1) return GPSA_EINVAL;
  if ((X2 == nullptr) != (d == nullptr)) return GPSA_EINVAL;
  gpsa::KmatBatch kb = gpsa::kmat_single();
  kb.axX = X2;
  kb.axd = d;
  kb.axs = (float)s;
  return gpsa::kmat_bwd_launch<float, double, double, float, double>(
      kind, Z, M, X, C, D, ls_u, var_u, Kbar, dZ, dX, dparams, 0, workspace, workspace_bytes, as_stream(stream), 1, kb);
}

}
```

spatial_alignment_amd/csrc/step.hip:

```cpp
#include <stdint.h>
#include <stdio.h>
#include <stdlib.h>
#include <string.h>

#include <new>
#include <vector>

#include "internal.hpp"

namespace gpsa {

constexpr int MAXMODS = GPSA_MAX_MODS;
constexpr int KM_MAXB_STEP = 16;

struct Arena {
  char* base = nullptr;
  long long off = 0, high = 0;
  long long limit = -1;
  bool dry = false;
  bool overflow = false;
  template <typename T>
  T* get(long long n) {
    off = (off + 255) & ~255LL;
    T* p = dry ? nullptr : reinterpret_cast<T*>(base + off);
// ... 373 lines not shown
      if (which == 1 && a.dvar_ws != nullptr) gsum += a.dvar_ws[b];
    }
    float* dst = which == 0 ? a.out.warp_ls : a.out.warp_var;
    if (dst != nullptr) dst[v] = (float)gsum;
    return;
  }
  e -= 2LL * a.V;
  const long long nG = (long long)a.Mg * D;
  if (e < nG) {
    double gsum = a.dZ_du[e];
    for (int p = 0; p < a.npass; ++p) gsum += a.dZ_df[(long long)p * nG + e];
    if (a.out.Gtilde != nullptr) a.out.Gtilde[e] = (float)gsum;
    return;
  }
  e -= nG;
  if (e < 2) {
    double gsum = a.dpar_du[e];
    for (int p = 0; p < a.npass; ++p) {
      gsum += a.dpar_df[(long long)p * 2 + e];
      if (e == 1) gsum += a.dvar_ds[p];
    }
    float* dst = e == 0 ? a.out.data_ls : a.out.data_var;
    if (dst != nullptr) dst[0] = (float)gsum;
    return;
  }
  e -= 2;
  for (int m = 0; m < a.nm; ++m) {
    const long long cnt = (long long)a.Mg * a.L[m];
    if (e < cnt) {
      if (a.out.delta_F[m] == nullptr) return;
      const int i = (int)(e / a.L[m]), l = (int)(e - (long long)i * a.L[m]);
      double gsum = a.ddc_F[m] != nullptr ? (double)a.ddc_F[m][e] : 0.0;
      if (a.dD_d != nullptr) gsum += a.dD_d[((long long)a.Loff[m] + l) * a.Mg + i];
      a.out.delta_F[m][e] = (float)gsum;
      return;
    }
    e -= cnt;
  }
}

constexpr int ADAM_MAXT = 16;
struct AdamArgs {
  float* p[ADAM_MAXT];
  const float* g[ADAM_MAXT];
  float* m[ADAM_MAXT];
  float* v[ADAM_MAXT];
  long long blk0[ADAM_MAXT + 1];
  long long n[ADAM_MAXT];
  int nt;
  double lr, b1, b2, eps;
};

__global__ void adam_tick_kernel(float* step) { step[0] += 1.f; }

__global__ void __launch_bounds__(256) adam_kernel(AdamArgs a, const float* __restrict__ step) {
  int t = 0;
  while (t + 1 < a.nt && (long long)blockIdx.x >= a.blk0[t + 1]) ++t;
  const double tt = (double)step[0];
  const float step_size = (float)(a.lr / (1.0 - pow(a.b1, tt))), rs2 = (float)sqrt(1.0 - pow(a.b2, tt));
  const float w1 = (float)(1.0 - a.b1), b2 = (float)a.b2, w2 = (float)(1.0 - a.b2), eps = (float)a.eps;
  const long long base = ((long long)blockIdx.x - a.blk0[t]) * 1024;
#pragma unroll
  for (int u = 0; u < 4; ++u) {
    const long long i = base + u * 256 + threadIdx.x;
    if (i < a.n[t]) {
      const float g = a.g[t][i];
      float m = a.m[t][i], v = a.v[t][i];
      m = m + w1 * (g - m);
      v = b2 * v + w2 * g * g;
      a.m[t][i] = m;
      a.v[t][i] = v;
      const float denom = sqrtf(v) / rs2 + eps;
      a.p[t][i] = a.p[t][i] - step_size * (m / denom);
    }
  }
}

struct Group {
  int M = 0, n_prior = 0, n_omega = 0, kl_off = 0;
  long long o_mats = 0, o_inv = 0, o_logdet = 0, o_info = 0, o_D = 0, o_KD = 0;
  int *om_idx = nullptr, *pr_idx = nullptr, *pr_list = nullptr, *grp_off = nullptr, *order = nullptr;
  int own_lo = 0, own_hi = 0;
  bool own_all() const { return own_lo == 0 && own_hi == n_omega; }
  int nb() const { return n_prior + n_omega; }
};

struct Run { int v0, b0, cnt; };

struct Pass {
  int m = 0;
  bool test = false;
  long long C = 0;
  long long o_alpha = 0, o_sigma = 0;
  long long o_keep = -1;
  long long o_alpha64 = -1;
  long long o_fuse = -1;
  bool x3 = false;
  bool gx3 = false;
  bool fused(const gpsa_step_io& io) const { return io.fuse_elbo != 0 && o_fuse >= 0 && io.Y[m] != nullptr; }
};

struct Plan {
  gpsa_step_desc d;
  std::vector<int> fixed;
  std::vector<long long> rows;
  int V, D, S, Mx, Mg, nm, nf;
  std::vector<int> free_views, bidx;
  std::vector<long long> nview, epsoff;
  long long Cs = 0, eps_total = 0;
  std::vector<Run> runs;
  bool merged = false;
  int ng = 0;
  Group grp[2];
  int Loff[MAXMODS], Ltot = 0;
  std::vector<Pass> passes;
  long long o_klcache = 0;
  long long o_resid = 0, o_Xv = 0, o_alpha_w = 0, o_Wk = 0, o_G64[MAXMODS], o_bad = 0, saved_bytes = 0;
  long long saved_bytes_nokeep = 0;
  long long o_apk_w = 0, o_apk_d = 0;
  long long nbad = 0;
  long long scratch_bytes = 0;
  long long bwd_acc_bytes = 0;
  char* dev = nullptr;
  ViewTab tab;
  int* d_free = nullptr;
  std::vector<hipEvent_t> tev;
  bool skip_seen = false;
  int lik[GPSA_MAX_MODS] = {};
  const float* log_offset[GPSA_MAX_MODS] = {};
  int tslots = 0, tfwd = 0, tbwd = 0;
  void tick(int kernel, int edge, bool fwd, hipStream_t st) {
    if (tslots == 0) return;
    const int slot = (fwd ? tfwd : tbwd) % tslots;
    (void)hipEventRecord(tev[(size_t)(slot * 3 + kernel) * 2 + edge], st);
  }

  struct GraphKey {
    static constexpr size_t O_IO = sizeof(gpsa_step_params), O_OG = O_IO + sizeof(gpsa_step_io),
                            O_PG = O_OG + sizeof(gpsa_step_out_grads), O_PTR = O_PG + sizeof(gpsa_step_param_grads),
                            BYTES = O_PTR + 3 * sizeof(void*) + 2 * sizeof(int);
    unsigned char b[BYTES];
    int stages() const { int v; memcpy(&v, b + O_PTR + 3 * sizeof(void*), sizeof(int)); return v; }
    int bwd() const { int v; memcpy(&v, b + O_PTR + 3 * sizeof(void*) + sizeof(int), sizeof(int)); return v; }
    void set(const gpsa_step_params* prm, const gpsa_step_io* io, const gpsa_step_out_grads* og,
             const gpsa_step_param_grads* pg, const void* saved, const void* scratch, const void* stream, int stages_,
             int bwd_) {
      memset(b, 0, BYTES);
      memcpy(b, prm, sizeof(*prm));
      memcpy(b + O_IO, io, sizeof(*io));
      if (og) memcpy(b + O_OG, og, sizeof(*og));
      if (pg) memcpy(b + O_PG, pg, sizeof(*pg));
      const void* ptrs[3] = {saved, scratch, stream};
      memcpy(b + O_PTR, ptrs, sizeof(ptrs));
      const int tail[2] = {stages_, bwd_};
      memcpy(b + O_PTR + sizeof(ptrs), tail, sizeof(tail));
    }
  };
  struct GraphEntry {
    GraphKey key;
    hipGraphExec_t exec;
    unsigned long long used;
    hipStream_t last;
  };
  std::vector<GraphEntry> graphs;
  struct Retired {
    hipGraphExec_t exec;
// ... 137 lines not shown
  for (int m = 0; m < nm; ++m) p->o_G64[m] = take((long long)S * dsc->n_rows[m] * D * 8);
  p->nbad = 0;
  for (int m = 0; m < nm; ++m) p->nbad += (dsc->n_rows[m] + 255) / 256;
  p->o_bad = take((p->nbad + 1) * 4);
  for (auto& q : p->passes) {
    q.o_alpha = take((long long)p->Mg * q.C * 4);
    q.o_sigma = take((long long)dsc->n_latent[q.m] * q.C * 4);
    if (dsc->exact_inducing_grad) q.o_alpha64 = take((long long)p->Mg * q.C * 8);
    const int Lq = dsc->n_latent[q.m];
    if (!q.test && !dsc->has_lmc[q.m] && gpsa_quadform_elbo_f32_workspace(p->Mg, q.C, Lq) > 0) {
      q.o_fuse = take((2LL * Lq + 1 + p->Mg) * q.C * 4);
      q.x3 = dsc->contraction == 1 && gpsa_quadform_elbo_x3_f32_workspace(p->Mg, q.C, Lq) > 0;
    }
    q.gx3 = !q.test && dsc->contraction == 1 && gpsa_quadform_bwd_omega_x3_workspace(p->Mg, q.C, Lq) > 0;
  }
  p->o_apk_w = take(gpsa_whiten_workspace(p->Mx) * (long long)(p->nf > 0 ? p->nf : 1));
  p->o_apk_d = take(gpsa_whiten_workspace(p->Mg));
  p->saved_bytes_nokeep = o + 256;
  {
    static const double keep_gb = [] { const char* e = getenv("GPSA_KEEP_GB"); return e ? atof(e) : 48.0; }();
    double budget = keep_gb * 1073741824.0;
    if (dsc->keep_budget_bytes > 0) {
      budget = (double)dsc->keep_budget_bytes;
    } else if (dsc->keep_budget_bytes < 0) {
      budget = -1.0;
    } else if (!host_only) {
      size_t fr = 0, total = 0;
      if (hipMemGetInfo(&fr, &total) == hipSuccess && 0.6 * (double)fr < budget) budget = 0.6 * (double)fr;
    }
    long long tot = 0;
    bool ok = true;
    for (auto& q : p->passes) {
      const long long b = gpsa_quadform_keep_f32_bytes(p->Mg, q.C, dsc->n_latent[q.m]);
      if (b == 0) ok = false;
      tot += b;
    }
    if (ok && (double)tot <= budget)
      for (auto& q : p->passes) q.o_keep = take(gpsa_quadform_keep_f32_bytes(p->Mg, q.C, dsc->n_latent[q.m]));
  }
  p->saved_bytes = o + 256;
  const long long n_ll = (long long)nm * (V + 1) + (long long)nm * V + V + V;
  long long n_int = V  + p->nf ;
  for (int g = 0; g < p->ng; ++g) {
    const Group& G = p->grp[g];
    n_int += 2 * G.n_omega + G.n_prior + (G.n_prior + 2) + G.n_omega;
  }
  const long long bytes = n_ll * 8 + n_int * 4 + 64;
  std::vector<char> host((size_t)bytes, 0);
  long long* hl = reinterpret_cast<long long*>(host.data());
  int* hi = reinterpret_cast<int*>(host.data() + n_ll * 8);
  if (!host_only && hipMalloc(reinterpret_cast<void**>(&p->dev), (size_t)bytes) != hipSuccess) { p->dev = nullptr; free_plan(p); return nullptr; }
  long long* dl = reinterpret_cast<long long*>(p->dev);
  int* di = reinterpret_cast<int*>(p->dev + n_ll * 8);
  long long lo = 0, io = 0;
  p->tab.vstart = dl + lo;
  for (int m = 0; m < nm; ++m) {
    long long acc = 0;
    for (int v = 0; v <= V; ++v) {
      hl[lo++] = acc;
      if (v < V) acc += p->rows[(long long)m * V + v];
    }
  }
  p->tab.colbase = dl + lo;
  for (int m = 0; m < nm; ++m)
    for (int v = 0; v < V; ++v) {
      long long acc = 0;
      for (int mm = 0; mm < m; ++mm) acc += p->rows[(long long)mm * V + v];
      hl[lo++] = acc;
    }
  p->tab.nview = dl + lo;
  for (int v = 0; v < V; ++v) hl[lo++] = p->nview[v];
  p->tab.epsoff = dl + lo;
  for (int v = 0; v < V; ++v) hl[lo++] = p->epsoff[v];
  p->tab.bidx = di + io;
  for (int v = 0; v < V; ++v) hi[io++] = p->bidx[v];
  p->d_free = di + io;
  for (int b = 0; b < p->nf; ++b) hi[io++] = p->free_views[b];
  for (int g = 0; g < p->ng; ++g) {
    Group& G = p->grp[g];
    std::vector<int> prior(G.n_omega, -1);
    for (int t = 0; t < G.n_omega; ++t) {
      if (g == 0 && t < V * D) prior[t] = p->bidx[t % V];
      else prior[t] = p->merged ? p->nf : 0;
      if (t < G.own_lo || t >= G.own_hi) prior[t] = -1;
    }
    G.om_idx = di + io;
    for (int t = 0; t < G.n_omega; ++t) hi[io++] = G.n_prior + t;
    G.pr_idx = di + io;
    for (int t = 0; t < G.n_omega; ++t) hi[io++] = prior[t];
    G.pr_list = di + io;
    for (int q = 0; q < G.n_prior; ++q) hi[io++] = q;
    std::vector<int> order, off(1, 0);
    for (int q = 0; q <= G.n_prior; ++q) {
      const int want = q < G.n_prior ? q : -1;
      for (int t = 0; t < G.n_omega; ++t)
        if (prior[t] == want) order.push_back(t);
      off.push_back((int)order.size());
    }
    G.grp_off = di + io;
    for (int q = 0; q < G.n_prior + 2; ++q) hi[io++] = off[q];
    G.order = di + io;
    for (int t = 0; t < G.n_omega; ++t) hi[io++] = order[t];
  }
  if (!host_only && hipMemcpy(p->dev, host.data(), (size_t)bytes, hipMemcpyHostToDevice) != hipSuccess) { free_plan(p); return nullptr; }
  p->tab.V = V; p->tab.D = D; p->tab.S = S; p->tab.nm = nm; p->tab.nf = p->nf; p->tab.Cs = p->Cs;
  return p;
}

static inline int splitk_for(long long k, int m, int n) {
  const long long tiles = cdiv(m, 64) * cdiv(n, 64);
  long long s = cdiv(512, tiles > 0 ? tiles : 1);
  if (s > 256) s = 256;
  if (s > k / 64) s = k / 64;
  if (s < 1) s = 1;
  return (int)s;
}
static inline int splitk_small(long long k, int m, int n, int batch) {
  if (batch == 1 && k >= 128 && k <= 1024 && cdiv(m, 64) * cdiv(n, 64) <= 32) {
    int s = (int)(k / 48);
    return s > 4 ? 4 : (s < 1 ? 1 : s);
  }
  return 1;
}

static inline int splitk_few(long long k, int m, int n, int batch) {
  if (batch <= 4 && k >= 128 && k <= 1024 && cdiv(m, 64) * cdiv(n, 64) * batch <= 64) {
    int s = (int)(k / 48);
    return s > 4 ? 4 : (s < 1 ? 1 : s);
  }
  return splitk_small(k, m, n, batch);
}

struct Ctx {
  Plan& P;
  const gpsa_step_params& prm;
  const gpsa_step_io& io;
  char* saved;
  Arena& sc;
  hipStream_t st;
  bool dry;
  bool apk_d = false;
  bool quiet = false;
  void* stv() const { return (void*)st; }
  template <typename T> T* sv(long long off) const { return reinterpret_cast<T*>(saved + off); }
  double* mats(const Group& G, int pos) const { return sv<double>(G.o_mats) + (long long)pos * G.M * G.M; }
  double* inv(const Group& G, int pos) const { return sv<double>(G.o_inv) + (long long)pos * G.M * G.M; }
};

static int gemm64(Ctx& c, int ta, int tb, int m, int n, long long k, double alpha, const double* A, long long lda,
                  long long sA, const double* B, long long ldb, long long sB, double beta, double* C,
                  long long ldc, long long sC, int batch, int splitk) {
  const bool dry = c.dry;
  const long long mk = c.sc.mark();
  void* ws = nullptr;
  long long wsb = 0;
  if (splitk > 1) {
    wsb = (long long)batch * splitk * m * n * 8;
    ws = c.sc.get<char>(wsb);
  }
  GPSA_RUN(gemm_launch<double>(ta, tb, m, n, k, alpha, A, lda, sA, B, ldb, sB, beta, C, ldc, sC, batch, splitk,
                               ws, wsb, c.st));
  c.sc.release(mk);
  return 0;
}
static int gemm32(Ctx& c, int ta, int tb, int m, int n, long long k, double alpha, const float* A, long long lda,
                  long long sA, const float* B, long long ldb, long long sB, double beta, float* C,
                  long long ldc, long long sC, int batch, int splitk) {
  const bool dry = c.dry;
  const long long mk = c.sc.mark();
  void* ws = nullptr;
  long long wsb = 0;
  if (splitk > 1) {
    wsb = (long long)batch * splitk * m * n * 4;
    ws = c.sc.get<char>(wsb);
  }
  GPSA_RUN(gemm_launch<float>(ta, tb, m, n, k, alpha, A, lda, sA, B, ldb, sB, beta, C, ldc, sC, batch, splitk,
                              ws, wsb, c.st));
  c.sc.release(mk);
  return 0;
}
static int thin_update(Ctx& c, const float* A, int M, int L, const float* B, long long C, float* out) {
  if (!c.dry) {
    if (c.sc.overflow) return GPSA_EWORKSPACE;
    const int rc = gpsa_thin_update_f32(A, M, L, B, C, out, c.stv());
    if (rc != GPSA_EUNSUPPORTED) return rc;
  }
  return gemm32(c, 0, 0, M, (int)C, L, 1.0, A, L, 0, B, C, 0, 1.0, out, C, 0, 1, 1);
}
template <typename TIA, typename TIB, typename TO>
static int gemmx(Ctx& c, int ta, int tb, int m, int n, long long k, double alpha, const TIA* A, long long lda,
                 long long sA, const TIB* B, long long ldb, long long sB, double beta, TO* C, long long ldc,
                 long long sC, int batch, int splitk) {
  const bool dry = c.dry;
  const long long mk = c.sc.mark();
  void* ws = nullptr;
  long long wsb = 0;
  if (splitk > 1) {
    wsb = (long long)batch * splitk * m * n * 8;
    ws = c.sc.get<char>(wsb);
  }
  GPSA_RUN((gemm64_launch<TIA, TIB, TO>(ta, tb, m, n, k, alpha, A, lda, sA, B, ldb, sB, beta, C, ldc, sC, batch,
                                        splitk, ws, wsb, c.st)));
  c.sc.release(mk);
  return 0;
}

static int longk(Ctx& c, int nprob, const double* const* G, const double* const* Bm, const void* const* d, int d_dtype,
                 int M, long long K, long long ld, int sym, const double* alpha, const double* beta, double* const* out) {
  const long long wsb = gpsa_longk_f64_workspace(M, K, nprob);
  if (wsb == 0 || (ld & 1)) return GPSA_EUNSUPPORTED;
  const long long mk = c.sc.mark();
  void* ws = c.sc.get<char>(wsb);
  int rc = 0;
  if (!c.dry) rc = gpsa_longk_f64(nprob, G, Bm, d, d_dtype, M, K, ld, sym, alpha, beta, out, ws, wsb, c.stv());
  c.sc.release(mk);
  return rc;
}

static int mm_stage_fwd(Ctx& c) {
  Plan& P = c.P;
  const bool dry = c.dry;
  const int V = P.V, D = P.D, Mx = P.Mx, Mg = P.Mg;
  Group& GW = P.gw();
  Group& GD = P.gd();
  const bool kl = P.d.want_kl != 0;
  double* klpart[2] = {nullptr, nullptr};
  int* klcnt[2] = {nullptr, nullptr};
  if (kl && !c.io.reuse_mm)
    for (int g = 0; g < P.ng; ++g)
      if (P.grp[g].n_omega > 0) {
        klpart[g] = c.sc.get<double>((long long)P.grp[g].n_omega * mvn_kl_grouped_fwd_slices(P.grp[g].M));
        klcnt[g] = c.sc.get<int>(P.grp[g].n_omega);
      }
  {
    PrepArgs a;
    memset(&a, 0, sizeof(a));
    a.Xtilde = c.prm.Xtilde; a.delta_G = c.prm.delta_G; a.slopes = c.prm.slopes; a.intercepts = c.prm.intercepts;
    for (int m = 0; m < P.nm; ++m) { a.delta_F[m] = c.prm.delta_F[m]; a.L[m] = P.d.n_latent[m]; a.Loff[m] = P.Loff[m]; }
    a.V = V; a.D = D; a.Mx = Mx; a.Mg = Mg; a.nm = P.nm;
    a.bidx = P.tab.bidx;
    a.mu_z = c.io.mu_z;
    a.resid = c.sv<double>(P.o_resid);
    a.Dw = kl ? c.sv<double>(GW.o_D) : nullptr;
    a.Dd = kl ? c.sv<double>(GD.o_D) + (P.merged ? (long long)V * D * Mx : 0) : nullptr;
    for (int g = 0; g < P.ng; ++g)
      if (kl && !P.grp[g].own_all() && !c.io.reuse_mm) {
        a.zinfo[g] = c.sv<int>(P.grp[g].o_info);
        a.nzinfo[g] = P.grp[g].nb();
      }
    for (int g = 0; g < P.ng; ++g)
      if (klcnt[g] != nullptr) {
        a.zinfo[2 + g] = klcnt[g];
        a.nzinfo[2 + g] = P.grp[g].n_omega;
      }
    const long long nd = kl ? cdiv((long long)P.Ltot * Mg, 256) : 0;
    if (!dry) {
      step_prep_kernel<<<(unsigned)(V + nd), 256, 0, c.st>>>(a);
      GPSA_LAUNCH_CHECK();
    }
  }
  if (c.io.reuse_mm) {
    if (kl && !dry)
      GPSA_CK(copy_async(c.io.kl, c.sv<double>(P.o_klcache), (size_t)((long long)V * D + P.Ltot) * 8, c.st));
    return 0;
  }
  for (const Run& r : P.runs)
    GPSA_RUN(gpsa_kmat_batched(P.d.kind_warp, c.prm.Xtilde + (long long)r.v0 * Mx * D, (long long)Mx * D, Mx,
                               c.prm.Xtilde + (long long)r.v0 * Mx * D, (long long)Mx * D, Mx, D,
                               c.prm.warp_ls + r.v0, c.prm.warp_var + r.v0, 1, nullptr, r.cnt, 1e-5,
                               c.mats(GW, P.pos_Kw(r.b0)), (long long)Mx * Mx, c.stv()));
  GPSA_RUN(gpsa_kmat_batched(P.d.kind_data, c.prm.Gtilde, 0, Mg, c.prm.Gtilde, 0, Mg, D, c.prm.data_ls,
                             c.prm.data_var, 0, nullptr, 1, 1e-5, c.mats(GD, P.pos_KF()), 0, c.stv()));
  const int m_first = (Mx == Mg && P.nm > 0) ? 1 : 0;
  if (m_first)
    GPSA_RUN(gpsa_omega_fwd2(c.prm.Omega_sqt_G, V * D, c.mats(GW, P.pos_OmG(0)), c.prm.Omega_sqt_F[0], P.d.n_latent[0],
                             c.mats(GD, P.pos_OmF(0, 0)), Mx, 1e-5, c.stv()));
  else
    GPSA_RUN(gpsa_omega_fwd(c.prm.Omega_sqt_G, Mx, V * D, 1e-5, c.mats(GW, P.pos_OmG(0)), c.stv()));
  for (int m = m_first; m < P.nm; ++m)
    GPSA_RUN(gpsa_omega_fwd(c.prm.Omega_sqt_F[m], Mg, P.d.n_latent[m], 1e-5, c.mats(GD, P.pos_OmF(m, 0)), c.stv()));
  for (int g = 0; g < P.ng; ++g) {
    Group& G = P.grp[g];
    const long long mm = (long long)G.M * G.M;
    double* logdet = c.sv<double>(G.o_logdet);
    int* info = c.sv<int>(G.o_info);
    const int np = G.n_prior, n_own = G.own_hi - G.own_lo;
    const bool sel = kl && !G.own_all();
    const int nb_main = kl ? G.nb() : np;
    auto inverse_product = [&](const double* Lin, double* out, int cnt) -> int {
      if (cnt <= 0) return 0;
      if (splitk_small(G.M, G.M, G.M, cnt) == 1)
        GPSA_RUN(gemm_launch_tri<double>(1, 0, G.M, G.M, G.M, 1.0, Lin, G.M, mm, Lin, G.M, mm, 0.0, out, G.M, mm, cnt, 1,
                                         nullptr, 0, c.st, GEMM_TRI_LTL));
      else
        GPSA_CK(gemm64(c, 1, 0, G.M, G.M, G.M, 1.0, Lin, G.M, mm, Lin, G.M, mm, 0.0, out, G.M, mm, cnt,
                       splitk_small(G.M, G.M, G.M, cnt)));
      return 0;
    };
    if (nb_main > 0) {
      const long long mk = c.sc.mark();
      double* Linv = c.sc.get<double>(nb_main * mm);
      if (G.M > 256) {
        const long long wsb = gpsa_chol_inv_blocked_workspace(G.M, nb_main);
        void* ws = c.sc.get<char>(wsb);
        if (!sel) {
          GPSA_RUN(gpsa_chol_inv_blocked_f64(c.mats(G, 0), Linv, G.M, nb_main, logdet, info, ws, wsb, c.stv()));
        } else {
          if (np > 0)
            GPSA_RUN(gpsa_chol_inv_blocked_f64(c.mats(G, 0), Linv, G.M, np, logdet, info, ws, wsb, c.stv()));
          if (n_own > 0)
            GPSA_RUN(gpsa_chol_inv_blocked_f64(c.mats(G, np + G.own_lo), Linv + (long long)(np + G.own_lo) * mm, G.M,
                                               n_own, logdet + np + G.own_lo, info + np + G.own_lo, ws, wsb, c.stv()));
        }
      } else if (!sel) {
        GPSA_RUN(gpsa_chol_inv_f64(c.mats(G, 0), Linv, G.M, nb_main, logdet, info, c.stv()));
      } else {
        GPSA_RUN(gpsa_chol_inv_sel_f64(c.mats(G, 0), Linv, G.M, nb_main, np, np + G.own_lo, np + G.own_hi, logdet, info,
                                       c.stv()));
      }
      if (!sel) {
        GPSA_CK(inverse_product(Linv, c.inv(G, 0), nb_main));
      } else if (G.own_lo == 0) {
        GPSA_CK(inverse_product(Linv, c.inv(G, 0), np + n_own));
      } else {
        GPSA_CK(inverse_product(Linv, c.inv(G, 0), np));
        GPSA_CK(inverse_product(Linv + (long long)(np + G.own_lo) * mm, c.inv(G, np + G.own_lo), n_own));
      }
      c.sc.release(mk);
    }
  }
  if (kl)
    for (int g = 0; g < P.ng; ++g) {
      Group& G = P.grp[g];
      if (G.n_omega > 0)
        GPSA_RUN(mvn_kl_grouped_fwd_copy(c.mats(G, 0), c.inv(G, 0), c.sv<double>(G.o_logdet), G.om_idx, G.pr_idx,
                                         c.sv<double>(G.o_D), G.M, G.n_omega, c.io.kl + G.kl_off,
                                         c.sv<double>(G.o_KD), c.sv<double>(P.o_klcache) + G.kl_off, klpart[g], klcnt[g],
                                         c.st));
    }
  return 0;
}

static ModPtrs mod_ptrs(Ctx& c, const gpsa_step_out_grads* og, const double* const* dG64) {
  ModPtrs p;
  memset(&p, 0, sizeof(p));
  for (int m = 0; m < c.P.nm; ++m) {
    p.X[m] = c.io.X[m];
    p.Gm[m] = c.io.G_means[m];
    p.Gs[m] = c.io.G_samples[m];
    p.G64[m] = c.sv<double>(c.P.o_G64[m]);
    p.N[m] = c.P.d.n_rows[m];
    if (og != nullptr) {
      p.dGm[m] = og->dG_means[m];
      p.dGs[m] = og->dG_samples[m];
    }
// ... 175 lines not shown
                                                 c.io.Y[m], (long long)(C / P.S), P.S, c.io.noise_u[m], g_ext, dmeanT, abar,
                                                 c.io.ll_part[m], c.io.F_fused_T[m], P.log_offset[m], skip ? 1 : 0, ws,
                                                 wsb, c.stv()));
    else if (pois)
      GPSA_RUN(gpsa_quadform_elbo_pois_f32(GPSA_F64, alpha, Om, Mg, C, L, meanT, q, c.prm.data_var, eps, c.io.Y[m],
                                           (long long)(C / P.S), P.S, c.io.noise_u[m], g_ext, dmeanT, abar,
                                           c.io.ll_part[m], c.io.F_fused_T[m], P.log_offset[m], skip ? 1 : 0, ws, wsb,
                                           c.stv()));
    else if (skip && mean_in_product)
      GPSA_RUN(gpsa_quadform_elbo_delta_skip_f32(GPSA_F64, alpha, Om, Mg, C, L, c.prm.delta_F[m], q, c.prm.data_var, eps,
                                                 c.io.Y[m], (long long)(C / P.S), P.S, c.io.noise_u[m], g_ext, dmeanT, abar,
                                                 c.io.ll_part[m], c.io.F_fused_T[m], ws, wsb, c.stv()));
    else if (skip)
      GPSA_RUN(gpsa_quadform_elbo_skip_f32(GPSA_F64, alpha, Om, Mg, C, L, meanT, q, c.prm.data_var, eps, c.io.Y[m],
                                           (long long)(C / P.S), P.S, c.io.noise_u[m], g_ext, dmeanT, abar,
                                           c.io.ll_part[m], c.io.F_fused_T[m], ws, wsb, c.stv()));
    else if (x3 && mean_in_product)
      GPSA_RUN(gpsa_quadform_elbo_delta_x3_f32(GPSA_F64, alpha, Om, Mg, C, L, c.prm.delta_F[m], q, c.prm.data_var, eps,
                                               c.io.Y[m], (long long)(C / P.S), P.S, c.io.noise_u[m], g_ext, dmeanT, abar,
                                               c.io.ll_part[m], c.io.F_fused_T[m], ws, wsb, c.stv()));
    else if (x3)
      GPSA_RUN(gpsa_quadform_elbo_x3_f32(GPSA_F64, alpha, Om, Mg, C, L, meanT, q, c.prm.data_var, eps, c.io.Y[m],
                                         (long long)(C / P.S), P.S, c.io.noise_u[m], g_ext, dmeanT, abar, c.io.ll_part[m],
                                         c.io.F_fused_T[m], ws, wsb, c.stv()));
    else if (mean_in_product)
      GPSA_RUN(gpsa_quadform_elbo_delta_f32(GPSA_F64, alpha, Om, Mg, C, L, c.prm.delta_F[m], q, c.prm.data_var, eps,
                                            c.io.Y[m], (long long)(C / P.S), P.S, c.io.noise_u[m], g_ext, dmeanT, abar,
                                            c.io.ll_part[m], c.io.F_fused_T[m], ws, wsb, c.stv()));
    else
      GPSA_RUN(gpsa_quadform_elbo_f32(GPSA_F64, alpha, Om, Mg, C, L, meanT, q, c.prm.data_var, eps, c.io.Y[m],
                                      (long long)(C / P.S), P.S, c.io.noise_u[m], g_ext, dmeanT, abar, c.io.ll_part[m],
                                      c.io.F_fused_T[m], ws, wsb, c.stv()));
    if (timed) { P.tick(0, 1, true, c.st); ++P.tfwd; }
    c.sc.release(mk);
    return 0;
  }
  {
    const long long wsb = gpsa_quadform_workspace(GPSA_F32, Mg, C, L);
    void* ws = c.sc.get<char>(wsb);
    const bool timed = !dry && !c.quiet && &ps == &P.passes[0];
    if (timed) P.tick(0, 0, true, c.st);
    if (c.io.keep_products && ps.o_keep >= 0)
      GPSA_RUN(gpsa_quadform_fwd_keep_f32(GPSA_F64, alpha, Om, Mg, C, L, v, c.sv<float>(ps.o_keep), ws, wsb, c.stv()));
    else
      GPSA_RUN(gpsa_quadform_fwd(GPSA_F32, GPSA_F64, alpha, Om, Mg, C, L, v, ws, wsb, c.stv()));
    if (timed) { P.tick(0, 1, true, c.st); ++P.tfwd; }
  }
  GPSA_RUN(gpsa_data_sample_fwd(meanT, v, q, c.prm.data_var, eps, C, L, F, Sigma, c.stv()));
  if (P.d.has_lmc[m] && Fo != nullptr)
    GPSA_CK(gemm32(c, 0, 0, (int)C, Pm, L, 1.0, F, L, 0, c.prm.W[m], Pm, 0, 0.0, Fo, Pm, 0, 1, 1));
  c.sc.release(mk);
  return 0;
}

static int step_forward(Plan& P, const gpsa_step_params& prm, const gpsa_step_io& io, char* saved, Arena& sc,
                        hipStream_t st, int stages) {
  Ctx c{P, prm, io, saved, sc, st, sc.dry};
  if (stages & 1) {
    GPSA_CK(mm_stage_fwd(c));
    GPSA_CK(warp_stage_fwd(c));
  }
  if (stages & 2) {
    const int mask = (stages >> 8) & ((1 << MAXMODS) - 1);
    c.quiet = (stages & 4) != 0;
    for (const Pass& ps : P.passes) {
      if (mask != 0 && (ps.test || ((mask >> ps.m) & 1) == 0)) continue;
      GPSA_CK(data_pass_fwd(c, ps));
    }
  }
  return 0;
}

struct BwdBufs {
  double* dstack[2];
  double *dZ_wf, *dZ_wu, *dpar_wf, *dpar_wu, *dvar_ws, *dresid;
  double *dZ_df, *dpar_df, *dZ_du, *dpar_du;
  double* dvar_ds;
  float* ddc_F[MAXMODS];
  double* dG64[MAXMODS];
  double* dD[2];
  bool have_dG[MAXMODS];
  bool have_ddc[MAXMODS];
  int* tick;
};
constexpr int BWD_TICKS = 64;

static int data_pass_bwd(Ctx& c, const Pass& ps, int pass_idx, const float* dFl_in, const float* dFo_in,
                         BwdBufs& B, const gpsa_step_param_grads& out, bool first_for_mod, const float* gloss) {
  Plan& P = c.P;
  const bool dry = c.dry;
  const int m = ps.m, Mg = P.Mg, D = P.D, L = P.d.n_latent[m], Pm = P.d.n_out[m];
  const long long C = ps.C, mm = (long long)Mg * Mg;
  Group& GD = P.gd();
  const double* Kinv = c.inv(GD, P.pos_KF());
  const double* Om = c.mats(GD, P.pos_OmF(m, 0));
  double* dOm = B.dstack[P.merged ? 0 : 1] + (long long)P.pos_OmF(m, 0) * mm;
  double* dKuu = B.dstack[P.merged ? 0 : 1] + (long long)P.pos_KF() * mm;
  const float* alpha = c.sv<float>(ps.o_alpha);
  const float* Sigma = c.sv<float>(ps.o_sigma);
  const float* eps = ps.test ? c.io.eps_F_test[m] : c.io.eps_F[m];
  const float* F = ps.test ? c.io.F_latent_test[m] : c.io.F_latent[m];
  const long long mk = c.sc.mark();
  const float* dFl = dFl_in;
  if (P.d.has_lmc[m] && dFo_in != nullptr) {
    float* buf = c.sc.get<float>(C * L);
    if (dFl_in != nullptr) GPSA_RUN(copy_async(buf, dFl_in, (size_t)(C * L * 4), c.st));
    GPSA_CK(gemm32(c, 0, 1, (int)C, L, Pm, 1.0, dFo_in, Pm, 0, c.prm.W[m], Pm, 0, dFl_in != nullptr ? 1.0 : 0.0, buf, L,
                   0, 1, 1));
    if (out.W[m] != nullptr)
      GPSA_CK(gemm32(c, 1, 0, L, Pm, C, 1.0, F, L, 0, dFo_in, Pm, 0, first_for_mod ? 0.0 : 1.0, out.W[m], Pm, 0, 1,
                     splitk_for(C, L, Pm)));
    dFl = buf;
  } else if (!P.d.has_lmc[m] && dFo_in != nullptr && dFl_in != nullptr && dFo_in != dFl_in) {
    return GPSA_EINVAL;
  } else if (dFl == nullptr) {
    dFl = dFo_in;
  }
  const bool fusedp = ps.fused(c.io);
  float* g_ext = fusedp ? c.sv<float>(ps.o_fuse) : c.sc.get<float>((long long)(L + 1) * C);
  float* dmeanT = fusedp ? g_ext + (long long)(L + 1) * C : c.sc.get<float>((long long)L * C);
  float* qbar = g_ext + (long long)L * C;
  if (!fusedp) {
    const long long wsb = 8 * (C / 32 + 2);
    void* ws = c.sc.get<char>(wsb);
    GPSA_RUN(gpsa_data_sample_bwd(dFl, eps, Sigma, c.prm.data_var, C, L, g_ext, dmeanT, qbar, GPSA_F64,
                                  B.dvar_ds + pass_idx, ws, wsb, c.stv()));
  }
  float* abar = fusedp ? dmeanT + (long long)L * C : c.sc.get<float>((long long)Mg * C);
  if (fusedp) {
    if (gloss == nullptr) return GPSA_EINVAL;
    const long long wsb = 8 * (C / 256 + 2);
    void* ws = c.sc.get<char>(wsb);
    const bool timed = !dry && !c.quiet && &ps == &P.passes[0];
    if (timed) P.tick(1, 0, false, c.st);
    if (pass_idx < BWD_TICKS - 32)
      GPSA_RUN(elbo_fused_post_ticket(g_ext, dmeanT, abar, Mg, C, L, gloss, c.prm.data_var, B.dvar_ds + pass_idx,
                                      (double*)ws, B.tick + 32 + pass_idx, c.st));
    else
      GPSA_RUN(gpsa_elbo_fused_post(g_ext, dmeanT, abar, Mg, C, L, gloss, c.prm.data_var, GPSA_F64,
                                    B.dvar_ds + pass_idx, ws, wsb, c.stv()));
    GPSA_CK(thin_update(c, c.prm.delta_F[m], Mg, L, dmeanT, C, abar));
    if (timed) P.tick(1, 1, false, c.st);
  } else {
    const long long wsb = gpsa_quadform_workspace(GPSA_F32, Mg, C, L);
    const long long mk2 = c.sc.mark();
    void* ws = c.sc.get<char>(wsb);
    const bool timed = !dry && !c.quiet && &ps == &P.passes[0];
    if (timed) P.tick(1, 0, false, c.st);
    const bool kept = c.io.keep_products && ps.o_keep >= 0;
    if (kept)
      GPSA_RUN(gpsa_quadform_bwd_alpha_kept_f32(c.sv<float>(ps.o_keep), g_ext, Mg, C, L, c.prm.delta_F[m], dmeanT, abar,
                                                c.stv()));
    else
      GPSA_RUN(gpsa_quadform_bwd_alpha(GPSA_F32, GPSA_F64, alpha, Om, g_ext, Mg, C, L, abar, ws, wsb, c.stv()));
    if (timed) P.tick(1, 1, false, c.st);
    c.sc.release(mk2);
    if (!kept) GPSA_CK(thin_update(c, c.prm.delta_F[m], Mg, L, dmeanT, C, abar));
  }
  const bool ddelta_in_gram = gpsa_quadform_bwd_omega_takes_delta(Mg, C) != 0;
  if (!ddelta_in_gram)
    GPSA_CK(gemm32(c, 0, 1, Mg, L, C, 1.0, alpha, C, 0, dmeanT, C, 0, first_for_mod ? 0.0 : 1.0, B.ddc_F[m], L, 0, 1,
                   splitk_for(C, Mg, L)));
  B.have_ddc[m] = true;
  const bool exact = ps.o_alpha64 >= 0;
  double* gamma64 = nullptr;
  if (exact) {
// ... 245 lines not shown
          be[i] = acc ? 1.0 : 0.0;
          os[i] = B.dstack[0] + (long long)P.pos_Kw(r.b0 + i) * mm;
        }
        rc = longk(c, r.cnt, Gs, Bs, ds, GPSA_F64, Mx, Cs, Cs, 0, al, be, os);
        if (rc != 0) return rc == GPSA_EUNSUPPORTED ? GPSA_EINVAL : rc;
        GPSA_RUN(gpsa_col_axpy_batched_f64(gamma + oMC, alpha + oMC, qbar + (long long)r.b0 * Cs, 2.0, Mx, Cs,
                                           gamma + oMC, r.cnt, c.stv()));
        done = true;
      } else if (rc != GPSA_EUNSUPPORTED) {
        return rc;
      }
    }
    if (!done || dry) {
      if (acc && !dry) return GPSA_EINVAL;
      {
        const long long mk2 = c.sc.mark();
        const long long wsb = gpsa_gram_batched_workspace(Mx, Cs, D, r.cnt);
        void* ws = c.sc.get<char>(wsb);
        GPSA_RUN(gpsa_gram_batched_f64(alpha + oMC, g + oDC, Mx, Cs, D, B.dstack[0] + (long long)P.pos_OmG(r.v0 * D) * mm,
                                       r.cnt, ws, wsb, c.stv()));
        c.sc.release(mk2);
      }
      GPSA_RUN(gpsa_col_axpy_batched_f64(gamma + oMC, alpha + oMC, qbar + (long long)r.b0 * Cs, 1.0, Mx, Cs, gamma + oMC,
                                         r.cnt, c.stv()));
      GPSA_CK(gemm64(c, 0, 1, Mx, Mx, Cs, -1.0, gamma + oMC, Cs, (long long)Mx * Cs, alpha + oMC, Cs, (long long)Mx * Cs,
                     0.0, B.dstack[0] + (long long)P.pos_Kw(r.b0) * mm, Mx, mm, r.cnt, splitk_for(Cs, Mx, Mx)));
      GPSA_RUN(gpsa_col_axpy_batched_f64(gamma + oMC, alpha + oMC, qbar + (long long)r.b0 * Cs, 1.0, Mx, Cs, gamma + oMC,
                                         r.cnt, c.stv()));
    }
    {
      const long long mk2 = c.sc.mark();
      long long nlive[KM_MAXB_STEP];
      for (int i = 0; i < r.cnt; ++i) nlive[i] = P.nview[r.v0 + i];
      const long long wsb = gpsa_kmat_bwd_batched_workspace(Mx, Cs, D, r.cnt);
      void* ws = c.sc.get<char>(wsb);
      GPSA_RUN(gpsa_kmat_bwd_batched(P.d.kind_warp, c.prm.Xtilde + (long long)r.v0 * Mx * D, (long long)Mx * D, Mx,
                                     Xv + (long long)r.b0 * Cs * D, Cs * D, Cs, D, c.prm.warp_ls + r.v0,
                                     c.prm.warp_var + r.v0, 1, nlive, r.cnt, gamma + oMC, (long long)Mx * Cs, 0,
                                     B.dZ_wf + (long long)r.b0 * Mx * D, (long long)Mx * D,
                                     B.dpar_wf + (long long)r.b0 * 2, ws, wsb, c.stv()));
      c.sc.release(mk2);
    }
  }
  c.sc.release(mk);
  return 0;
}

static bool warp_runs_longk(const Plan& P) {
  for (const Run& r : P.runs)
    if (!(r.cnt * P.D <= 48 && gpsa_longk_f64_workspace(P.Mx, P.Cs, r.cnt * P.D) > 0 &&
          gpsa_longk_f64_workspace(P.Mx, P.Cs, r.cnt) > 0))
      return false;
  return true;
}

static int step_backward(Plan& P, const gpsa_step_params& prm, const gpsa_step_io& io,
                         const gpsa_step_out_grads& og, char* saved, Arena& sc, const gpsa_step_param_grads& out,
                         hipStream_t st) {
  Ctx c{P, prm, io, saved, sc, st, sc.dry};
  const bool dry = c.dry;
  const int V = P.V, D = P.D, Mx = P.Mx, Mg = P.Mg, nf = P.nf, npass = (int)P.passes.size();
  BwdBufs B;
  memset(&B, 0, sizeof(B));
  const bool kl = P.d.want_kl != 0 && og.dkl != nullptr;
  for (int g = 0; g < P.ng; ++g) {
    Group& G = P.grp[g];
    B.dD[g] = sc.get<double>((long long)G.n_omega * G.M);
  }
  const long long z0 = (sc.off + 255) & ~255LL;
  for (int g = 0; g < P.ng; ++g) {
    Group& G = P.grp[g];
    B.dstack[g] = sc.get<double>((long long)G.nb() * G.M * G.M);
  }
  const long long nwz = (long long)(nf > 0 ? nf : 1) * Mx * D;
  B.dZ_wf = sc.get<double>(nwz);
  B.dpar_wf = sc.get<double>(2LL * (nf > 0 ? nf : 1));
  B.dvar_ws = sc.get<double>(nf > 0 ? nf : 1);
  B.dresid = sc.get<double>((long long)V * Mx * D);
  B.dZ_df = sc.get<double>((long long)(npass > 0 ? npass : 1) * Mg * D);
  B.dpar_df = sc.get<double>(2LL * (npass > 0 ? npass : 1));
  B.dvar_ds = sc.get<double>(npass > 0 ? npass : 1);
  B.tick = sc.get<int>(BWD_TICKS);
  const long long zf = sc.off;
  sc.get<char>(256);
  const long long z1 = (sc.off + 255) & ~255LL;
  if (!dry) GPSA_CK(zero_fill_async(sc.base + z0, (size_t)(z1 - z0), st));
  if (dry) {
    long long ab = z1 - z0;
    for (int m = 0; m < P.nm; ++m) ab += ((long long)Mg * P.d.n_latent[m] * 4 + 255) & ~255LL;
    for (int m = 0; m < P.nm; ++m)
      if (P.d.has_lmc[m]) ab += ((long long)P.d.n_latent[m] * P.d.n_out[m] * 4 + 255) & ~255LL;
    P.bwd_acc_bytes = ab + 256;
  }
  B.dZ_wu = sc.get<double>(nwz);
  B.dpar_wu = sc.get<double>(2LL * (nf > 0 ? nf : 1));
  B.dZ_du = sc.get<double>((long long)Mg * D); B.dpar_du = sc.get<double>(2);
  for (int m = 0; m < P.nm; ++m) {
    B.ddc_F[m] = sc.get<float>((long long)Mg * P.d.n_latent[m]);
    B.dG64[m] = sc.get<double>((long long)P.S * P.d.n_rows[m] * D);
  }
  bool seen[MAXMODS] = {false, false, false, false};
  for (int pi = 0; pi < npass; ++pi) {
    const Pass& ps = P.passes[pi];
    const float* dFl = ps.test ? og.dF_latent_test[ps.m] : og.dF_latent[ps.m];
    const float* dFo = ps.test ? og.dF_obs_test[ps.m] : og.dF_obs[ps.m];
    if (dFl == nullptr && dFo == nullptr && !ps.fused(io)) continue;
    GPSA_CK(data_pass_bwd(c, ps, pi, dFl, dFo, B, out, !seen[ps.m], og.gloss));
    seen[ps.m] = true;
  }
  const bool early = io.f_event != nullptr && !dry && (io.bwd_acc == nullptr || io.bwd_acc_mode == 0) &&
                     warp_runs_longk(P);
  if (!early) GPSA_CK(warp_stage_bwd(c, og, B, false));
  if (io.bwd_acc_mode != 0 && io.bwd_acc != nullptr && !dry) {
    char* accb = reinterpret_cast<char*>(io.bwd_acc);
    const long long nD = (zf - z0) / 8;
    double* rD = reinterpret_cast<double*>(sc.base + z0);
    double* aD = reinterpret_cast<double*>(accb);
    long long aoff = z1 - z0;
    if (io.bwd_acc_mode == 1) {
      GPSA_CK(copy_async(aD, rD, (size_t)(nD * 8), st));
    } else {
      double* dst = io.bwd_acc_mode == 2 ? aD : rD;
      const double* src = io.bwd_acc_mode == 2 ? rD : aD;
      add_inplace_kernel<<<(unsigned)cdiv(nD, 256), 256, 0, st>>>(dst, src, nD);
      GPSA_LAUNCH_CHECK();
    }
    for (int m = 0; m < P.nm; ++m) {
      const long long n = (long long)Mg * P.d.n_latent[m];
      float* a = reinterpret_cast<float*>(accb + aoff);
      aoff += (n * 4 + 255) & ~255LL;
      if (!B.have_ddc[m]) {
        if (io.bwd_acc_mode == 1) GPSA_CK(zero_fill_async(a, (size_t)(n * 4), st));
        continue;
      }
      if (io.bwd_acc_mode == 1) {
        GPSA_CK(copy_async(a, B.ddc_F[m], (size_t)(n * 4), st));
      } else {
        add_inplace_f32_kernel<<<(unsigned)cdiv(n, 256), 256, 0, st>>>(io.bwd_acc_mode == 2 ? a : B.ddc_F[m],
                                                                        io.bwd_acc_mode == 2 ? B.ddc_F[m] : a, n);
        GPSA_LAUNCH_CHECK();
      }
    }
    for (int m = 0; m < P.nm; ++m) {
      if (!P.d.has_lmc[m]) continue;
      const long long n = (long long)P.d.n_latent[m] * P.d.n_out[m];
      float* a = reinterpret_cast<float*>(accb + aoff);
      aoff += (n * 4 + 255) & ~255LL;
      if (out.W[m] == nullptr) continue;
      if (io.bwd_acc_mode == 1) {
        GPSA_CK(copy_async(a, out.W[m], (size_t)(n * 4), st));
      } else {
        add_inplace_f32_kernel<<<(unsigned)cdiv(n, 256), 256, 0, st>>>(io.bwd_acc_mode == 2 ? a : out.W[m],
                                                                        io.bwd_acc_mode == 2 ? out.W[m] : a, n);
        GPSA_LAUNCH_CHECK();
      }
    }
    if (io.bwd_acc_mode != 3) return 0;
  }
  auto kl_backward = [&]() -> int {
    for (int g = 0; g < P.ng && kl; ++g) {
      Group& G = P.grp[g];
      if (G.n_omega == 0 || G.n_prior == 0) continue;
      const long long mm = (long long)G.M * G.M;
      const long long mk = sc.mark();
      double* S = sc.get<double>((long long)G.n_prior * mm);
      double* T1 = sc.get<double>((long long)G.n_prior * mm);
      GPSA_RUN(gpsa_mvn_kl_grouped_bwd_acc(c.mats(G, 0), c.inv(G, 0), G.om_idx, G.pr_list, G.grp_off, G.order,
                                           c.sv<double>(G.o_D), c.sv<double>(G.o_KD), og.dkl + G.kl_off, G.M, G.n_omega,
                                           G.n_prior, B.dstack[g] + (long long)G.n_prior * mm, B.dD[g], S, 1, c.stv()));
      GPSA_CK(gemm64(c, 0, 0, G.M, G.M, G.M, 1.0, c.inv(G, 0), G.M, mm, S, G.M, mm, 0.0, T1, G.M, mm, G.n_prior,
                     splitk_few(G.M, G.M, G.M, G.n_prior)));
      GPSA_CK(gemm64(c, 0, 0, G.M, G.M, G.M, 0.5, T1, G.M, mm, c.inv(G, 0), G.M, mm, 1.0, B.dstack[g], G.M, mm, G.n_prior,
                     splitk_few(G.M, G.M, G.M, G.n_prior)));
      sc.release(mk);
    }
    return 0;
  };
  auto priors_backward = [&]() -> int {
    {
      for (const Run& r : P.runs) {
        const long long mk = sc.mark();
        const long long wsb = gpsa_kmat_bwd_batched_workspace(Mx, Mx, D, r.cnt);
        void* ws = sc.get<char>(wsb);
        GPSA_RUN(gpsa_kmat_bwd_batched(P.d.kind_warp, prm.Xtilde + (long long)r.v0 * Mx * D, (long long)Mx * D, Mx,
                                       prm.Xtilde + (long long)r.v0 * Mx * D, (long long)Mx * D, Mx, D, prm.warp_ls + r.v0,
                                       prm.warp_var + r.v0, 1, nullptr, r.cnt,
                                       B.dstack[0] + (long long)P.pos_Kw(r.b0) * Mx * Mx, (long long)Mx * Mx, 1,
                                       B.dZ_wu + (long long)r.b0 * Mx * D, (long long)Mx * D, B.dpar_wu + (long long)r.b0 * 2,
                                       ws, wsb, c.stv()));
        sc.release(mk);
      }
      {
        const long long mk = sc.mark();
        const long long wsb = gpsa_kmat_bwd_batched_workspace(Mg, Mg, D, 1);
        void* ws = sc.get<char>(wsb);
        GPSA_RUN(gpsa_kmat_bwd_batched(P.d.kind_data, prm.Gtilde, 0, Mg, prm.Gtilde, 0, Mg, D, prm.data_ls, prm.data_var, 0,
                                       nullptr, 1, B.dstack[P.merged ? 0 : 1] + (long long)P.pos_KF() * Mg * Mg, 0, 1,
                                       B.dZ_du, 0, B.dpar_du, ws, wsb, c.stv()));
        sc.release(mk);
      }
    }
    return 0;
  };
  auto omega_backward = [&](int which) -> int {
    int m_first = 0;
    if ((which & 1) && out.Omega_sqt_G != nullptr) {
      if ((which & 2) && Mx == Mg && P.nm > 0 && out.Omega_sqt_F[0] != nullptr) {
        m_first = 1;
        GPSA_RUN(gpsa_omega_bwd2(B.dstack[0] + (long long)P.pos_OmG(0) * Mx * Mx, prm.Omega_sqt_G, out.Omega_sqt_G, V * D,
                                 B.dstack[P.merged ? 0 : 1] + (long long)P.pos_OmF(0, 0) * Mg * Mg, prm.Omega_sqt_F[0],
                                 out.Omega_sqt_F[0], P.d.n_latent[0], Mx, 1, c.stv()));
      } else {
        GPSA_RUN(gpsa_omega_bwd(B.dstack[0] + (long long)P.pos_OmG(0) * Mx * Mx, prm.Omega_sqt_G, Mx, V * D, 1,
                                out.Omega_sqt_G, c.stv()));
      }
    }
    if (which & 2)
      for (int m = m_first; m < P.nm; ++m)
        if (out.Omega_sqt_F[m] != nullptr)
          GPSA_RUN(gpsa_omega_bwd(B.dstack[P.merged ? 0 : 1] + (long long)P.pos_OmF(m, 0) * Mg * Mg, prm.Omega_sqt_F[m], Mg,
                                  P.d.n_latent[m], 1, out.Omega_sqt_F[m], c.stv()));
    return 0;
  };
  auto finalize = [&](int part) -> int {
    FinalArgs a;
    memset(&a, 0, sizeof(a));
    a.part = part;
    a.V = V; a.D = D; a.Mx = Mx; a.Mg = Mg; a.nm = P.nm; a.nf = nf; a.npass = npass;
    a.bidx = P.tab.bidx;
    a.slopes = prm.slopes;
    a.dZ_wf = B.dZ_wf; a.dZ_wu = B.dZ_wu; a.dpar_wf = B.dpar_wf; a.dpar_wu = B.dpar_wu; a.dvar_ws = B.dvar_ws;
    a.dresid = B.dresid;
    a.dD_w = kl ? B.dD[0] : nullptr;
    a.dZ_df = B.dZ_df; a.dpar_df = B.dpar_df; a.dvar_ds = B.dvar_ds; a.dZ_du = B.dZ_du; a.dpar_du = B.dpar_du;
    a.dD_d = kl ? (P.merged ? B.dD[0] + (long long)V * D * Mx : B.dD[1]) : nullptr;
    const long long nsmall = (long long)V * Mx * D + 2LL * V + (long long)Mg * D + 2;
    long long nF = 0;
    for (int m = 0; m < P.nm; ++m) {
      a.ddc_F[m] = B.have_ddc[m] ? B.ddc_F[m] : nullptr;
      a.L[m] = P.d.n_latent[m];
      a.Loff[m] = P.Loff[m];
      nF += (long long)Mg * P.d.n_latent[m];
    }
    a.out = out;
    if (part != 1 && io.loss_src != nullptr && io.loss_dst != nullptr) {
      a.loss_src = io.loss_src;
      a.loss_dst = io.loss_dst;
    }
    const long long tot = part == 1 ? nF : (part == 2 ? nsmall : nsmall + nF);
    if (!dry && tot > 0) {
      step_finalize_kernel<<<(unsigned)cdiv(tot, 256), 256, 0, st>>>(a);
      GPSA_LAUNCH_CHECK();
    }
    return 0;
  };
  if (early) {
    ++P.n_early;
    GPSA_CK(kl_backward());
    GPSA_CK(omega_backward(2));
    GPSA_CK(finalize(1));
    GPSA_CK((int)hipEventRecord(reinterpret_cast<hipEvent_t>(io.f_event), st));
    GPSA_CK(warp_stage_bwd(c, og, B, true));
// ... 385 lines not shown
```

spatial_alignment_amd/ops.py:

```python
import os

import torch

from . import _lib

F32, F64 = 0, 1
KINDS = {"rbf": 0, "matern12": 1, "matern32": 2}


def _dt(t):
    if t.dtype == torch.float32:
        return F32
    if t.dtype == torch.float64:
        return F64
    raise TypeError(f"unsupported dtype {t.dtype}")


def _p(t):
    return 0 if t is None else t.data_ptr()


_raw_stream = torch._C._cuda_getCurrentRawStream


# ... 515 lines not shown
                                      self._stream(F))
        _lib.check(rc, "gpsa_loglik_fwd")
        return out

    def loglik_bwd(self, F, Y, noise_u, gout):
        F, Y = self._c(F), self._c(Y)
        S, N, P = F.shape
        dF = torch.empty_like(F)
        dn = torch.empty(1, dtype=torch.float32, device=F.device)
        ws = self._ws(8 * 4100, F)
        rc = self.lib.gpsa_loglik_bwd(_p(F), _p(Y), _p(noise_u), _p(gout), S, N, P, _p(dF), _p(dn),
                                      _p(ws), ws.numel(), self._stream(F))
        _lib.check(rc, "gpsa_loglik_bwd")
        return dF, dn

    def bdot(self, A, B):
        nb = A.shape[0] if A.dim() == 3 else B.shape[0]
        A2 = self._c(A)
        B2 = self._c(B)
        n = A2.shape[-1] * A2.shape[-2]
        sA = n if A2.dim() == 3 else 0
        sB = n if B2.dim() == 3 else 0
        out = torch.empty(nb, dtype=A2.dtype, device=A2.device)
        ws = self._ws(8 * 32 * nb, A2)
        rc = self.lib.gpsa_bdot(_dt(A2), _p(A2), sA, _p(B2), sB, n, nb, _p(out), _p(ws), ws.numel(),
                                self._stream(A2))
        _lib.check(rc, "gpsa_bdot")
        return out

    @staticmethod
    def _lstride(t):
        M = t.shape[-1]
        if t.stride(-1) == 1 and t.stride(-2) == M:
            return t, t.stride(0)
        t = t.contiguous()
        return t, M * M

    def mvn_kl_fwd(self, Kinv, logdetK, Omega, logdetO, Dm):
        Omega, so = self._lstride(Omega)
        L, M = Omega.shape[0], Omega.shape[-1]
        Kinv, Dm = self._c(Kinv), self._c(Dm)
        kl = torch.empty(L, dtype=torch.float64, device=Kinv.device)
        KD = self.gemm(Kinv, Dm)
        rc = self.lib.gpsa_mvn_kl_fwd(_p(Kinv), _p(logdetK), _p(Omega), so, _p(logdetO), logdetO.stride(0),
                                      _p(Dm), _p(KD), M, L, _p(kl), self._stream(Kinv))
        _lib.check(rc, "gpsa_mvn_kl_fwd")
        return kl, KD

    def mvn_kl_bwd(self, Kuu, Kinv, Omega, Oinv, Dm, KD, g):
        Omega, so = self._lstride(Omega)
        Oinv, si = self._lstride(Oinv)
        L, M = Omega.shape[0], Omega.shape[-1]
        Kuu, Kinv, Dm, KD, g = self._c(Kuu), self._c(Kinv), self._c(Dm), self._c(KD), self._c(g)
        dev = Kinv.device
        dOm = torch.empty(L, M, M, dtype=torch.float64, device=dev)
        dDm = torch.empty(M, L, dtype=torch.float64, device=dev)
        Sp = torch.empty(M, M, dtype=torch.float64, device=dev)
        rc = self.lib.gpsa_mvn_kl_bwd(_p(Kuu), _p(Kinv), _p(Omega), so, _p(Oinv), si, _p(Dm), _p(KD), _p(g),
                                      M, L, _p(dOm), _p(dDm), _p(Sp), self._stream(Kinv))
        _lib.check(rc, "gpsa_mvn_kl_bwd")
        return dOm, dDm, Sp

    def mvn_kl_grouped_fwd(self, mats, inv, logdet, plan, D):
        T, M = D.shape
        kl = torch.empty(T, dtype=torch.float64, device=D.device)
        KD = torch.empty(T, M, dtype=torch.float64, device=D.device)
        rc = self.lib.gpsa_mvn_kl_grouped_fwd(_p(mats), _p(inv), _p(logdet), _p(plan.om_idx), _p(plan.pr_idx),
                                              _p(D), M, T, _p(kl), _p(KD), self._stream(D))
        _lib.check(rc, "gpsa_mvn_kl_grouped_fwd")
        return kl, KD

    def mvn_kl_grouped_bwd(self, mats, inv, plan, D, KD, g):
        T, M = D.shape
        dev = D.device
        dOm = torch.empty(T, M, M, dtype=torch.float64, device=dev)
        dD = torch.empty(T, M, dtype=torch.float64, device=dev)
        S = torch.empty(plan.P, M, M, dtype=torch.float64, device=dev)
        rc = self.lib.gpsa_mvn_kl_grouped_bwd(_p(mats), _p(inv), _p(plan.om_idx), _p(plan.pr_list),
                                              _p(plan.grp_off), _p(plan.order), _p(D), _p(KD), _p(g), M, T,
                                              plan.P, _p(dOm), _p(dD), _p(S), self._stream(D))
        _lib.check(rc, "gpsa_mvn_kl_grouped_bwd")
        return dOm, dD, S

    def elbo_fwd(self, ll, kl, kl_scale):
        ll, kl = self._c(ll), self._c(kl)
        loss = torch.empty(1, dtype=torch.float32, device=ll.device)
        rc = self.lib.gpsa_elbo_fwd(_p(ll), ll.numel(), _p(kl), kl.numel(), float(kl_scale), _p(loss),
                                    self._stream(ll))
        _lib.check(rc, "gpsa_elbo_fwd")
        return loss

    def elbo_bwd(self, gloss, n_ll, n_kl, kl_scale):
        gloss = self._f32(gloss.reshape(1))
        dll = torch.empty(n_ll, dtype=torch.float64, device=gloss.device)
        dkl = torch.empty(max(n_kl, 1), dtype=torch.float64, device=gloss.device)[:n_kl]
        rc = self.lib.gpsa_elbo_bwd(_p(gloss), n_ll, n_kl, float(kl_scale), _p(dll), _p(dkl),
                                    self._stream(gloss))
        _lib.check(rc, "gpsa_elbo_bwd")
        return dll, dkl

    def kmeans_assign(self, X, centres, want_d2=False):
        X, centres = self._c(X), self._c(centres)
        N, D = X.shape
        K = centres.shape[0]
        assign = torch.empty(N, dtype=torch.int32, device=X.device)
        d2 = torch.empty(N, dtype=torch.float32, device=X.device) if want_d2 else None
        rc = self.lib.gpsa_kmeans_assign(_p(X), N, D, _p(centres), K, _p(assign), _p(d2), self._stream(X))
        _lib.check(rc, "gpsa_kmeans_assign")
        return assign, d2

    def kmeans_update(self, X, assign, centres):
        X = self._c(X)
        assert centres.is_contiguous()
        N, D = X.shape
        K = centres.shape[0]
        counts = torch.empty(K, dtype=torch.int32, device=X.device)
        ws = self._ws(self.lib.gpsa_kmeans_workspace(N, D, K), X)
        rc = self.lib.gpsa_kmeans_update(_p(X), _p(assign), N, D, K, _p(centres), _p(counts), _p(ws),
                                         ws.numel(), self._stream(X))
        _lib.check(rc, "gpsa_kmeans_update")
        return counts

    def add_diag(self, A, s):
        assert A.is_contiguous()
        M = A.shape[-1]
        nb = A.numel() // (M * M)
        rc = self.lib.gpsa_add_diag(_dt(A), _p(A), M, nb, float(s), self._stream(A))
        _lib.check(rc, "gpsa_add_diag")
        return A


_ops = None


def get_ops():
    global _ops
    if _ops is None:
        _ops = HipOps()
    return _ops


def set_ops(obj):
    global _ops
    _ops = obj
```

Measured before the change: 150.5.

## Split KL backward over term slices and merge warp/data prior kernels into one launch

The grouped MVN-KL backward kernel can now split a prior group's terms into slices of 8 along grid z. Partial sums are written to a workspace, and the last-arriving block (tracked by an atomic tick counter) reduces them, so groups with many terms get more parallelism. Separately, the warp and data Kuu kernel matrices and their backward are computed in one batched launch by treating the data prior as an extra 'tail' batch entry, which saves launches. The cost is extra workspace, atomics and fence logic, plus a tick buffer that must be reset after each use.

Result: no change. 151.5 (median of 6 runs) (+0.6%).

```diff
diff --git a/include/gpsa_hip.h b/include/gpsa_hip.h
--- a/include/gpsa_hip.h
+++ b/include/gpsa_hip.h
@@ -199,6 +199,16 @@
                           const long long* n_live, int batch, const double* Kbar, long long strideK, int same,
                           double* dZ, long long stride_dZ, double* dparams, void* workspace,
                           long long workspace_bytes, void* stream);
+int gpsa_kmat_uu_tail_ok(int M, int D, int batch);
+int gpsa_kmat_uu_batched_tail(int kind, const float* Z, long long strideZ, int M, int D, const float* ls_u,
+                              const float* var_u, int stride_par, int batch, const float* Zt, const float* ls_t,
+                              const float* var_t, double jitter, double* K, long long strideK, double* Kt,
+                              void* stream);
+int gpsa_kmat_uu_bwd_batched_tail(int kind, const float* Z, long long strideZ, int M, int D, const float* ls_u,
+                                  const float* var_u, int stride_par, int batch, const float* Zt, const float* ls_t,
+                                  const float* var_t, const double* Kbar, long long strideK, const double* Kbar_t,
+                                  double* dZ, long long stride_dZ, double* dparams, double* dZ_t, double* dparams_t,
+                                  void* workspace, long long workspace_bytes, void* stream);
 int gpsa_kmat_bwd_x64(int kind, const float* Z, int M, const double* X, long long C, int D, const float* ls_u,
                       const float* var_u, const float* Kbar, double* dZ, double* dX, double* dparams,
                       void* workspace, long long workspace_bytes, void* stream);
@@ -246,6 +256,12 @@
                                 const int* pr_list, const int* grp_off, const int* order, const double* D,
                                 const double* KD, const double* g, int M, int T, int P, double* dOmega,
                                 double* dD, double* S, int accumulate, void* stream);
+long long gpsa_mvn_kl_grouped_bwd_sliced_workspace(int M, int P, int max_terms);
+int gpsa_mvn_kl_grouped_bwd_sliced(const double* mats, const double* inv, const int* om_idx,
+                                   const int* pr_list, const int* grp_off, const int* order, const double* D,
+                                   const double* KD, const double* g, int M, int T, int P, double* dOmega,
+                                   double* dD, double* S, int accumulate, int max_terms, void* ws,
+                                   long long ws_bytes, int* tick, long long n_tick, void* stream);
 
 #define GPSA_MAX_MODS 4
 
diff --git a/spatial_alignment_amd/_lib.py b/spatial_alignment_amd/_lib.py
--- a/spatial_alignment_amd/_lib.py
+++ b/spatial_alignment_amd/_lib.py
@@ -121,6 +121,10 @@
 SIGNATURES.update({
     "gpsa_kmat_batched": (_i, [_i, _vp, _ll, _i, _vp, _ll, _ll, _i, _vp, _vp, _i, C.POINTER(_ll), _i, _d, _vp, _ll, _vp]),
     "gpsa_kmat_bwd_batched_workspace": (_ll, [_i, _ll, _i, _i]),
+    "gpsa_kmat_uu_tail_ok": (_i, [_i, _i, _i]),
+    "gpsa_kmat_uu_batched_tail": (_i, [_i, _vp, _ll, _i, _i, _vp, _vp, _i, _i, _vp, _vp, _vp, _d, _vp, _ll, _vp, _vp]),
+    "gpsa_kmat_uu_bwd_batched_tail": (_i, [_i, _vp, _ll, _i, _i, _vp, _vp, _i, _i, _vp, _vp, _vp, _vp, _ll, _vp, _vp,
+                                           _ll, _vp, _vp, _vp, _vp, _ll, _vp]),
     "gpsa_kmat_bwd_batched": (_i, [_i, _vp, _ll, _i, _vp, _ll, _ll, _i, _vp, _vp, _i, C.POINTER(_ll), _i, _vp, _ll, _i,
                                    _vp, _ll, _vp, _vp, _ll, _vp]),
     "gpsa_kmat_bwd_x64": (_i, [_i, _vp, _i, _vp, _ll, _i, _vp, _vp, _vp, _vp, _vp, _vp, _vp, _ll, _vp]),
@@ -145,6 +149,9 @@
     "gpsa_gram_batched_f64": (_i, [_vp, _vp, _i, _ll, _i, _vp, _i, _vp, _ll, _vp]),
     "gpsa_mvn_kl_grouped_bwd_acc": (_i, [_vp, _vp, _vp, _vp, _vp, _vp, _vp, _vp, _vp, _i, _i, _i, _vp, _vp, _vp, _i,
                                          _vp]),
+    "gpsa_mvn_kl_grouped_bwd_sliced_workspace": (_ll, [_i, _i, _i]),
+    "gpsa_mvn_kl_grouped_bwd_sliced": (_i, [_vp, _vp, _vp, _vp, _vp, _vp, _vp, _vp, _vp, _i, _i, _i, _vp, _vp, _vp, _i,
+                                            _i, _vp, _ll, _vp, _ll, _vp]),
     "gpsa_step_create": (_vp, [C.POINTER(StepDesc)]),
     "gpsa_step_describe": (_i, [C.POINTER(StepDesc), C.POINTER(_ll)]),
     "gpsa_step_destroy": (None, [_vp]),
diff --git a/spatial_alignment_amd/csrc/internal.hpp b/spatial_alignment_amd/csrc/internal.hpp
--- a/spatial_alignment_amd/csrc/internal.hpp
+++ b/spatial_alignment_amd/csrc/internal.hpp
@@ -27,6 +27,13 @@
 int mvn_kl_grouped_fwd_copy(const double* mats, const double* inv, const double* logdet, const int* om_idx,
                             const int* pr_idx, const double* D, int M, int T, double* kl, double* KD,
                             double* kl_copy, double* part, int* cnt, hipStream_t st);
+
+int mvn_kl_grouped_bwd_slices(int max_terms);
+long long mvn_kl_grouped_bwd_blocks(int M);
+int mvn_kl_grouped_bwd_sliced(const double* mats, const double* inv, const int* om_idx, const int* pr_list,
+                              const int* grp_off, const int* order, const double* D, const double* KD, const double* g,
+                              int M, int T, int P, double* dOmega, double* dD, double* S, int accumulate, int slices,
+                              double* part, double* gsum, int* tick, hipStream_t st);
 
 int lmc_mfma_launch(const float* F, const float* W, const float* Y, const float* noise_u, int S, long long N, int L,
                     int P, double* zpart, int nparts, float* dF, float* dWpart, int G, hipStream_t st);
diff --git a/spatial_alignment_amd/csrc/kl.hip b/spatial_alignment_amd/csrc/kl.hip
--- a/spatial_alignment_amd/csrc/kl.hip
+++ b/spatial_alignment_amd/csrc/kl.hip
@@ -129,55 +129,108 @@
                           const int* __restrict__ order, const double* __restrict__ D,
                           const double* __restrict__ KD, const double* __restrict__ g, int M, int T, int P,
                           double* __restrict__ dOmega, double* __restrict__ dD, double* __restrict__ S,
-                          int accumulate) {
+                          int accumulate, double* part, double* gsum, int* tick) {
+  __shared__ int last_s;
   const long long mm = (long long)M * M, e = blockIdx.x * 256LL + threadIdx.x;
-  const int pg = blockIdx.y;
+  const bool live = e < mm;
+  const int pg = blockIdx.y, z = blockIdx.z;
   const int t0 = grp_off[pg], t1 = grp_off[pg + 1];
   if (pg == P) {
+    if (z != 0) return;
     if (blockIdx.x == 0)
       for (int q = t0; q < t1; ++q)
         for (int m = threadIdx.x; m < M; m += 256) dD[(long long)order[q] * M + m] = 0.0;
-    if (!accumulate && e < mm)
+    if (!accumulate && live)
       for (int q = t0; q < t1; ++q) dOmega[(long long)order[q] * mm + e] = 0.0;
     return;
   }
+  int nsl = (part != nullptr && t1 - t0 > 8) ? (t1 - t0 + 7) / 8 : 1;
+  if (nsl > (int)gridDim.z) nsl = (int)gridDim.z;
+  if (z >= nsl) return;
+  const int qa = nsl > 1 ? t0 + 8 * z : t0;
+  const int qb = (nsl > 1 && z < nsl - 1) ? qa + 8 : t1;
   const int p = pr_list[pg];
   if (blockIdx.x == 0)
-    for (int q = t0; q < t1; ++q) {
+    for (int q = qa; q < qb; ++q) {
       const int t = order[q];
       for (int m = threadIdx.x; m < M; m += 256) dD[(long long)t * M + m] = g[t] * KD[(long long)t * M + m];
     }
-  if (e >= mm) return;
-  const int i = (int)(e / M), j = (int)(e % M);
-  const double kinv = inv[(long long)p * mm + e];
   double s0 = 0.0, s1 = 0.0, gs = 0.0;
-  for (int q = t0; q < t1; q += 8) {
-    double ga[8], om[8], oi[8], di[8], dj[8], old[8];
-    int tt[8];
-#pragma unroll
-    for (int u = 0; u < 8; ++u) {
-      const bool on = q + u < t1;
-      const int ta = order[on ? q + u : t0];
-      tt[u] = on ? ta : -1;
-      ga[u] = on ? g[ta] : 0.0;
-      const long long mo = (long long)om_idx[ta] * mm + e;
-      om[u] = mats[mo];
-      oi[u] = inv[mo];
-      di[u] = D[(long long)ta * M + i];
-      dj[u] = D[(long long)ta * M + j];
-      old[u] = (accumulate && on) ? dOmega[(long long)ta * mm + e] : 0.0;
-    }
-#pragma unroll
-    for (int u = 0; u < 8; ++u)
-      if (tt[u] >= 0) dOmega[(long long)tt[u] * mm + e] = old[u] + 0.5 * ga[u] * (kinv - oi[u]);
-#pragma unroll
-    for (int u = 0; u < 8; u += 2) {
-      gs += ga[u] + ga[u + 1];
-      s0 += ga[u] * (om[u] + di[u] * dj[u]);
-      s1 += ga[u + 1] * (om[u + 1] + di[u + 1] * dj[u + 1]);
-    }
-  }
-  S[(long long)pg * mm + e] = gs * mats[(long long)p * mm + e] - (s0 + s1);
+  if (live) {
+    const int i = (int)(e / M), j = (int)(e % M);
+    const double kinv = inv[(long long)p * mm + e];
+    for (int q = qa; q < qb; q += 8) {
+      double ga[8], om[8], oi[8], di[8], dj[8], old[8];
+      int tt[8];
+#pragma unroll
+      for (int u = 0; u < 8; ++u) {
+        const bool on = q + u < qb;
+        const int ta = order[on ? q + u : t0];
+        tt[u] = on ? ta : -1;
+        ga[u] = on ? g[ta] : 0.0;
+        const long long mo = (long long)om_idx[ta] * mm + e;
+        om[u] = mats[mo];
+        oi[u] = inv[mo];
+        di[u] = D[(long long)ta * M + i];
+        dj[u] = D[(long long)ta * M + j];
+        old[u] = (accumulate && on) ? dOmega[(long long)ta * mm + e] : 0.0;
+      }
+#pragma unroll
+      for (int u = 0; u < 8; ++u)
+        if (tt[u] >= 0) dOmega[(long long)tt[u] * mm + e] = old[u] + 0.5 * ga[u] * (kinv - oi[u]);
+#pragma unroll
+      for (int u = 0; u < 8; u += 2) {
+        gs += ga[u] + ga[u + 1];
+        s0 += ga[u] * (om[u] + di[u] * dj[u]);
+        s1 += ga[u + 1] * (om[u + 1] + di[u + 1] * dj[u + 1]);
+      }
+    }
+  }
+  if (nsl == 1) {
+    if (live) S[(long long)pg * mm + e] = gs * mats[(long long)p * mm + e] - (s0 + s1);
+    return;
+  }
+  const long long NZ = gridDim.z, NX = gridDim.x;
+  if (live)
+    __hip_atomic_store(&part[((long long)pg * NZ + z) * mm + e], s0 + s1, __ATOMIC_RELAXED, __HIP_MEMORY_SCOPE_AGENT);
+  if (threadIdx.x == 0)
+    __hip_atomic_store(&gsum[((long long)pg * NZ + z) * NX + blockIdx.x], gs, __ATOMIC_RELAXED, __HIP_MEMORY_SCOPE_AGENT);
+  asm volatile("s_waitcnt vmcnt(0)" ::: "memory");
+  __syncthreads();
+  if (threadIdx.x == 0) {
+    last_s = atomicAdd(&tick[(long long)pg * NX + blockIdx.x], 1) == nsl - 1;
+    if (last_s) {
+      __builtin_amdgcn_fence(__ATOMIC_ACQUIRE, "agent");
+      asm volatile("s_waitcnt vmcnt(0)" ::: "memory");
+    }
+  }
+  __syncthreads();
+  if (!last_s) return;
+  if (live) {
+    double gt = 0.0, st = 0.0;
+    for (int zz = 0; zz < nsl; ++zz) {
+      gt += __hip_atomic_load(&gsum[((long long)pg * NZ + zz) * NX + blockIdx.x], __ATOMIC_RELAXED, __HIP_MEMORY_SCOPE_AGENT);
+      st += __hip_atomic_load(&part[((long long)pg * NZ + zz) * mm + e], __ATOMIC_RELAXED, __HIP_MEMORY_SCOPE_AGENT);
+    }
+    S[(long long)pg * mm + e] = gt * mats[(long long)p * mm + e] - st;
+  }
+  if (threadIdx.x == 0) tick[(long long)pg * NX + blockIdx.x] = 0;
+}
+
+int mvn_kl_grouped_bwd_slices(int max_terms) { return max_terms > 8 ? (max_terms + 7) / 8 : 1; }
+long long mvn_kl_grouped_bwd_blocks(int M) { return cdiv((long long)M * M, 256); }
+int mvn_kl_grouped_bwd_sliced(const double* mats, const double* inv, const int* om_idx, const int* pr_list,
+                              const int* grp_off, const int* order, const double* D, const double* KD, const double* g,
+                              int M, int T, int P, double* dOmega, double* dD, double* S, int accumulate, int slices,
+                              double* part, double* gsum, int* tick, hipStream_t st) {
+  if (M < 1 || T < 1 || P < 1 || slices < 1) return GPSA_EINVAL;
+  if (slices > 1 && (part == nullptr || gsum == nullptr || tick == nullptr)) return GPSA_EINVAL;
+  if (slices == 1) part = nullptr;
+  dim3 grid((unsigned)mvn_kl_grouped_bwd_blocks(M), (unsigned)(P + 1), (unsigned)slices);
+  mvn_kl_grouped_bwd_kernel<<<grid, 256, 0, st>>>(mats, inv, om_idx, pr_list, grp_off, order, D, KD, g, M, T, P, dOmega,
+                                                  dD, S, accumulate, part, gsum, tick);
+  GPSA_LAUNCH_CHECK();
+  return 0;
 }
 
 int mvn_kl_grouped_fwd_slices(int M) { return M > 64 ? (M + 63) / 64 < 8 ? (M + 63) / 64 : 8 : 1; }
@@ -213,9 +266,34 @@
   if (M < 1 || T < 1 || P < 1) return GPSA_EINVAL;
   dim3 grid((unsigned)cdiv((long long)M * M, 256), (unsigned)(P + 1));
   gpsa::mvn_kl_grouped_bwd_kernel<<<grid, 256, 0, as_stream(stream)>>>(
-      mats, inv, om_idx, pr_list, grp_off, order, D, KD, g, M, T, P, dOmega, dD, S, accumulate);
-  GPSA_LAUNCH_CHECK();
-  return 0;
+      mats, inv, om_idx, pr_list, grp_off, order, D, KD, g, M, T, P, dOmega, dD, S, accumulate, nullptr, nullptr, nullptr);
+  GPSA_LAUNCH_CHECK();
+  return 0;
+}
+
+long long gpsa_mvn_kl_grouped_bwd_sliced_workspace(int M, int P, int max_terms) {
+  if (M < 1 || P < 1) return 0;
+  const long long ns = gpsa::mvn_kl_grouped_bwd_slices(max_terms);
+  if (ns == 1) return 0;
+  return (long long)P * ns * ((long long)M * M + gpsa::mvn_kl_grouped_bwd_blocks(M)) * 8;
+}
+
+int gpsa_mvn_kl_grouped_bwd_sliced(const double* mats, const double* inv, const int* om_idx,
+                                   const int* pr_list, const int* grp_off, const int* order, const double* D,
+                                   const double* KD, const double* g, int M, int T, int P, double* dOmega,
+                                   double* dD, double* S, int accumulate, int max_terms, void* ws,
+                                   long long ws_bytes, int* tick, long long n_tick, void* stream) {
+  if (M < 1 || T < 1 || P < 1) return GPSA_EINVAL;
+  const int ns = gpsa::mvn_kl_grouped_bwd_slices(max_terms);
+  double *part = nullptr, *gsum = nullptr;
+  if (ns > 1) {
+    if (ws == nullptr || ws_bytes < gpsa_mvn_kl_grouped_bwd_sliced_workspace(M, P, max_terms)) return GPSA_EWORKSPACE;
+    if (tick == nullptr || n_tick < (long long)P * gpsa::mvn_kl_grouped_bwd_blocks(M)) return GPSA_EWORKSPACE;
+    part = static_cast<double*>(ws);
+    gsum = part + (long long)P * ns * M * M;
+  }
+  return gpsa::mvn_kl_grouped_bwd_sliced(mats, inv, om_idx, pr_list, grp_off, order, D, KD, g, M, T, P, dOmega, dD, S,
+                                         accumulate, ns, part, gsum, tick, as_stream(stream));
 }
 
 int gpsa_mvn_kl_grouped_bwd(const double* mats, const double* inv, const int* om_idx,
diff --git a/spatial_alignment_amd/csrc/kmat.hip b/spatial_alignment_amd/csrc/kmat.hip
--- a/spatial_alignment_amd/csrc/kmat.hip
+++ b/spatial_alignment_amd/csrc/kmat.hip
@@ -13,6 +13,9 @@
   const void* axX;
   const float* axd;
   float axs;
+  int tail;
+  const void *tZ, *tX, *tls, *tvar;
+  void* tK;
 };
 static inline KmatBatch kmat_single() {
   KmatBatch kb;
@@ -21,6 +24,9 @@
   kb.axX = nullptr;
   kb.axd = nullptr;
   kb.axs = 0.f;
+  kb.tail = -1;
+  kb.tZ = kb.tX = kb.tls = kb.tvar = nullptr;
+  kb.tK = nullptr;
   for (int i = 0; i < KM_MAXB; ++i) kb.n[i] = 0;
   return kb;
 }
@@ -32,11 +38,19 @@
                 T* __restrict__ K, KmatBatch kb) {
   __shared__ T Zs[KM_ROWS][MAXD];
   const int b = blockIdx.z;
-  Z += b * kb.sZ;
-  X += b * kb.sX;
-  K += b * kb.sK;
-  ls_u += b * kb.sP;
-  var_u += b * kb.sP;
+  if (b == kb.tail) {
+    Z = static_cast<const TI*>(kb.tZ);
+    X = static_cast<const TX*>(kb.tX);
+    K = static_cast<T*>(kb.tK);
+    ls_u = static_cast<const TI*>(kb.tls);
+    var_u = static_cast<const TI*>(kb.tvar);
+  } else {
+    Z += b * kb.sZ;
+    X += b * kb.sX;
+    K += b * kb.sK;
+    ls_u += b * kb.sP;
+    var_u += b * kb.sP;
+  }
   const long long live = kb.ragged ? kb.n[b] : C;
   const int m0 = blockIdx.y * KM_ROWS;
   if (threadIdx.x < KM_ROWS * MAXD) {
@@ -85,11 +99,19 @@
                 T* __restrict__ spart, KmatBatch bt) {
   {
     const long long b = blockIdx.z;
-    Z += b * bt.sZ;
-    X += b * bt.sX;
-    Kbar += b * bt.sK;
-    ls_u += b * bt.sP;
-    var_u += b * bt.sP;
+    if (b == bt.tail) {
+      Z = static_cast<const TI*>(bt.tZ);
+      X = static_cast<const TX*>(bt.tX);
+      Kbar = static_cast<const TK*>(bt.tK);
+      ls_u = static_cast<const TI*>(bt.tls);
+      var_u = static_cast<const TI*>(bt.tvar);
+    } else {
+      Z += b * bt.sZ;
+      X += b * bt.sX;
+      Kbar += b * bt.sK;
+      ls_u += b * bt.sP;
+      var_u += b * bt.sP;
+    }
     zpart += b * (long long)gridDim.x * M * D;
     if (xpart != nullptr) xpart += b * (long long)gridDim.y * C * D;
     spart += b * (long long)gridDim.x * gridDim.y * 2;
@@ -166,11 +188,19 @@
   static_assert(MCH % 8 == 0, "the closing reduction takes 8 rows at a time");
   {
     const long long b = blockIdx.z;
-    Z += b * bt.sZ;
-    X += b * bt.sX;
-    Kbar += b * bt.sK;
-    ls_u += b * bt.sP;
-    var_u += b * bt.sP;
+    if (b == bt.tail) {
+      Z = static_cast<const TI*>(bt.tZ);
+      X = static_cast<const TX*>(bt.tX);
+      Kbar = static_cast<const TK*>(bt.tK);
+      ls_u = static_cast<const TI*>(bt.tls);
+      var_u = static_cast<const TI*>(bt.tvar);
+    } else {
+      Z += b * bt.sZ;
+      X += b * bt.sX;
+      Kbar += b * bt.sK;
+      ls_u += b * bt.sP;
+      var_u += b * bt.sP;
+    }
     zpart += b * (long long)gridDim.x * M * D;
     if (xpart != nullptr) xpart += b * (long long)gridDim.y * C * D;
     spart += b * (long long)gridDim.x * gridDim.y * 2;
@@ -293,15 +323,21 @@
 kmat_bwd_finish_kernel(const T* __restrict__ zpart, long long nbx, long long nz,
                        const T* __restrict__ xpart, long long nby, long long nx,
                        const T* __restrict__ spart, long long ns, int same, TO* __restrict__ dZ,
-                       TO* __restrict__ dX, TO* __restrict__ dparams, long long sdZ, long long sdX) {
+                       TO* __restrict__ dX, TO* __restrict__ dparams, long long sdZ, long long sdX, int tail,
+                       TO* __restrict__ tdZ, TO* __restrict__ tdparams) {
   {
     const long long b = blockIdx.y;
     zpart += b * nbx * nz;
     if (xpart != nullptr) xpart += b * nby * nx;
     spart += b * ns * 2;
-    dZ += b * sdZ;
-    if (dX != nullptr) dX += b * sdX;
-    dparams += b * 2;
+    if (b == tail) {
+      dZ = tdZ;
+      dparams = tdparams;
+    } else {
+      dZ += b * sdZ;
+      if (dX != nullptr) dX += b * sdX;
+      dparams += b * 2;
+    }
   }
   __shared__ double red[256];
   const long long zb = (nz + 15) / 16, xb = (nx + 63) / 64;
@@ -373,8 +409,9 @@
 int kmat_bwd_launch(int kind, const TI* Z, int M, const TX* X, long long C, int D, const TI* ls_u,
                     const TI* var_u, const TK* Kbar, TO* dZ, TO* dX, TO* dparams, int same, void* ws,
                     long long ws_bytes, hipStream_t st, int batch = 1, KmatBatch kb = kmat_single(),
-                    long long sdZ = 0, long long sdX = 0) {
+                    long long sdZ = 0, long long sdX = 0, TO* tdZ = nullptr, TO* tdparams = nullptr) {
   if (batch < 1 || batch > KM_MAXB) return GPSA_EINVAL;
+  if (kb.tail >= 0 && (kb.tail >= batch || dX != nullptr || tdZ == nullptr || tdparams == nullptr)) return GPSA_EINVAL;
   const int mch = kb_rows(M, C * batch);
   const long long ncb = cdiv(C, 256), nby = cdiv(M, mch);
   long long nbx = ncb < KB_MAXBX ? ncb : KB_MAXBX;
@@ -415,7 +452,8 @@
     if (fold2 && (nx != nz)) return GPSA_EINVAL;
     dim3 fgrid2((unsigned)(cdiv(nz, 16) + cdiv(nx, 64) + 1), (unsigned)batch);
     kmat_bwd_finish_kernel<T, TO><<<fgrid2, 256, 0, st>>>(zpart, nbx, nz, xp, nby2, nx, spart, nbx * nby2,
-                                                          fold2 ? 1 : 0, dZ, dX, dparams, sdZ, sdX);
+                                                          fold2 ? 1 : 0, dZ, dX, dparams, sdZ, sdX, kb.tail, tdZ,
+                                                          tdparams);
     GPSA_LAUNCH_CHECK();
     return 0;
   }
@@ -441,7 +479,7 @@
   if (fold && (nx != nz)) return GPSA_EINVAL;
   dim3 fgrid((unsigned)(cdiv(nz, 16) + cdiv(nx, 64) + 1), (unsigned)batch);
   kmat_bwd_finish_kernel<T, TO><<<fgrid, 256, 0, st>>>(zpart, nbx, nz, xp, nby, nx, spart, nbx * nby,
-                                                       fold ? 1 : 0, dZ, dX, dparams, sdZ, sdX);
+                                                       fold ? 1 : 0, dZ, dX, dparams, sdZ, sdX, kb.tail, tdZ, tdparams);
   GPSA_LAUNCH_CHECK();
   return 0;
 }
@@ -548,6 +586,44 @@
       as_stream(stream), batch, make_batch(strideZ, strideX, strideK, stride_par, n_live, batch), stride_dZ, 0);
 }
 
+int gpsa_kmat_uu_tail_ok(int M, int D, int batch) {
+  return D == 2 && M >= 1 && M <= 256 && batch >= 1 && batch + 1 <= gpsa::KM_MAXB;
+}
+
+int gpsa_kmat_uu_batched_tail(int kind, const float* Z, long long strideZ, int M, int D, const float* ls_u,
+                              const float* var_u, int stride_par, int batch, const float* Zt, const float* ls_t,
+                              const float* var_t, double jitter, double* K, long long strideK, double* Kt,
+                              void* stream) {
+  if (D < 1 || D > gpsa::MAXD || M < 1 || batch < 1 || batch + 1 > gpsa::KM_MAXB) return GPSA_EINVAL;
+  if (Zt == nullptr || ls_t == nullptr || var_t == nullptr || Kt == nullptr) return GPSA_EINVAL;
+  gpsa::KmatBatch kb = make_batch(strideZ, strideZ, strideK, stride_par, nullptr, batch);
+  kb.tail = batch;
+  kb.tZ = kb.tX = Zt;
+  kb.tls = ls_t;
+  kb.tvar = var_t;
+  kb.tK = Kt;
+  return gpsa::kmat_launch<float, float, double>(kind, Z, M, Z, M, D, ls_u, var_u, jitter, K, as_stream(stream),
+                                                 batch + 1, kb);
+}
+
+int gpsa_kmat_uu_bwd_batched_tail(int kind, const float* Z, long long strideZ, int M, int D, const float* ls_u,
+                                  const float* var_u, int stride_par, int batch, const float* Zt, const float* ls_t,
+                                  const float* var_t, const double* Kbar, long long strideK, const double* Kbar_t,
+                                  double* dZ, long long stride_dZ, double* dparams, double* dZ_t, double* dparams_t,
+                                  void* workspace, long long workspace_bytes, void* stream) {
+  if (!gpsa_kmat_uu_tail_ok(M, D, batch)) return GPSA_EUNSUPPORTED;
+  if (Zt == nullptr || ls_t == nullptr || var_t == nullptr || Kbar_t == nullptr) return GPSA_EINVAL;
+  gpsa::KmatBatch kb = make_batch(strideZ, strideZ, strideK, stride_par, nullptr, batch);
+  kb.tail = batch;
+  kb.tZ = kb.tX = Zt;
+  kb.tls = ls_t;
+  kb.tvar = var_t;
+  kb.tK = const_cast<double*>(Kbar_t);
+  return gpsa::kmat_bwd_launch<float, double, double, double, float>(
+      kind, Z, M, Z, M, D, ls_u, var_u, Kbar, dZ, (double*)nullptr, dparams, 1, workspace, workspace_bytes,
+      as_stream(stream), batch + 1, kb, stride_dZ, 0, dZ_t, dparams_t);
+}
+
 int gpsa_kmat_bwd_x64(int kind, const float* Z, int M, const double* X, long long C, int D, const float* ls_u,
                       const float* var_u, const float* Kbar, double* dZ, double* dX, double* dparams,
                       void* workspace, long long workspace_bytes, void* stream) {
diff --git a/spatial_alignment_amd/csrc/step.hip b/spatial_alignment_amd/csrc/step.hip
--- a/spatial_alignment_amd/csrc/step.hip
+++ b/spatial_alignment_amd/csrc/step.hip
@@ -479,6 +479,8 @@
   int *om_idx = nullptr, *pr_idx = nullptr, *pr_list = nullptr, *grp_off = nullptr, *order = nullptr;
   int own_lo = 0, own_hi = 0;
   bool own_all() const { return own_lo == 0 && own_hi == n_omega; }
+  int kl_max_terms = 0;
+  int kl_max_terms_all = 0;
   int nb() const { return n_prior + n_omega; }
 };
 
@@ -782,8 +784,15 @@
     for (int t = 0; t < G.n_omega; ++t) {
       if (g == 0 && t < V * D) prior[t] = p->bidx[t % V];
       else prior[t] = p->merged ? p->nf : 0;
+    }
+    {
+      std::vector<int> cnt(G.n_prior > 0 ? G.n_prior : 1, 0);
+      G.kl_max_terms_all = 0;
+      for (int t = 0; t < G.n_omega; ++t)
+        if (prior[t] >= 0 && ++cnt[prior[t]] > G.kl_max_terms_all) G.kl_max_terms_all = cnt[prior[t]];
+    }
+    for (int t = 0; t < G.n_omega; ++t)
       if (t < G.own_lo || t >= G.own_hi) prior[t] = -1;
-    }
     G.om_idx = di + io;
     for (int t = 0; t < G.n_omega; ++t) hi[io++] = G.n_prior + t;
     G.pr_idx = di + io;
@@ -799,6 +808,9 @@
     }
     G.grp_off = di + io;
     for (int q = 0; q < G.n_prior + 2; ++q) hi[io++] = off[q];
+    G.kl_max_terms = 0;
+    for (int q = 0; q < G.n_prior; ++q)
+      if (off[q + 1] - off[q] > G.kl_max_terms) G.kl_max_terms = off[q + 1] - off[q];
     G.order = di + io;
     for (int t = 0; t < G.n_omega; ++t) hi[io++] = order[t];
   }
@@ -917,6 +929,11 @@
   return rc;
 }
 
+static bool priors_one_launch(const Plan& P) {
+  return P.runs.size() == 1 && P.d.kind_warp == P.d.kind_data && P.Mx == P.Mg &&
+         gpsa_kmat_uu_tail_ok(P.Mx, P.D, P.runs[0].cnt) != 0;
+}
+
 static int mm_stage_fwd(Ctx& c) {
   Plan& P = c.P;
   const bool dry = c.dry;
@@ -964,13 +981,21 @@
       GPSA_CK(copy_async(c.io.kl, c.sv<double>(P.o_klcache), (size_t)((long long)V * D + P.Ltot) * 8, c.st));
     return 0;
   }
-  for (const Run& r : P.runs)
-    GPSA_RUN(gpsa_kmat_batched(P.d.kind_warp, c.prm.Xtilde + (long long)r.v0 * Mx * D, (long long)Mx * D, Mx,
-                               c.prm.Xtilde + (long long)r.v0 * Mx * D, (long long)Mx * D, Mx, D,
-                               c.prm.warp_ls + r.v0, c.prm.warp_var + r.v0, 1, nullptr, r.cnt, 1e-5,
-                               c.mats(GW, P.pos_Kw(r.b0)), (long long)Mx * Mx, c.stv()));
-  GPSA_RUN(gpsa_kmat_batched(P.d.kind_data, c.prm.Gtilde, 0, Mg, c.prm.Gtilde, 0, Mg, D, c.prm.data_ls,
-                             c.prm.data_var, 0, nullptr, 1, 1e-5, c.mats(GD, P.pos_KF()), 0, c.stv()));
+  if (priors_one_launch(P)) {
+    const Run& r = P.runs[0];
+    GPSA_RUN(gpsa_kmat_uu_batched_tail(P.d.kind_warp, c.prm.Xtilde + (long long)r.v0 * Mx * D, (long long)Mx * D, Mx, D,
+                                       c.prm.warp_ls + r.v0, c.prm.warp_var + r.v0, 1, r.cnt, c.prm.Gtilde,
+                                       c.prm.data_ls, c.prm.data_var, 1e-5, c.mats(GW, P.pos_Kw(r.b0)),
+                                       (long long)Mx * Mx, c.mats(GD, P.pos_KF()), c.stv()));
+  } else {
+    for (const Run& r : P.runs)
+      GPSA_RUN(gpsa_kmat_batched(P.d.kind_warp, c.prm.Xtilde + (long long)r.v0 * Mx * D, (long long)Mx * D, Mx,
+                                 c.prm.Xtilde + (long long)r.v0 * Mx * D, (long long)Mx * D, Mx, D,
+                                 c.prm.warp_ls + r.v0, c.prm.warp_var + r.v0, 1, nullptr, r.cnt, 1e-5,
+                                 c.mats(GW, P.pos_Kw(r.b0)), (long long)Mx * Mx, c.stv()));
+    GPSA_RUN(gpsa_kmat_batched(P.d.kind_data, c.prm.Gtilde, 0, Mg, c.prm.Gtilde, 0, Mg, D, c.prm.data_ls,
+                               c.prm.data_var, 0, nullptr, 1, 1e-5, c.mats(GD, P.pos_KF()), 0, c.stv()));
+  }
   const int m_first = (Mx == Mg && P.nm > 0) ? 1 : 0;
   if (m_first)
     GPSA_RUN(gpsa_omega_fwd2(c.prm.Omega_sqt_G, V * D, c.mats(GW, P.pos_OmG(0)), c.prm.Omega_sqt_F[0], P.d.n_latent[0],
@@ -1312,6 +1337,7 @@
   bool have_dG[MAXMODS];
   bool have_ddc[MAXMODS];
   int* tick;
+  int* kl_tick[2];
 };
 constexpr int BWD_TICKS = 64;
 
@@ -1723,6 +1749,11 @@
   B.dvar_ds = sc.get<double>(npass > 0 ? npass : 1);
   B.tick = sc.get<int>(BWD_TICKS);
   const long long zf = sc.off;
+  for (int g = 0; g < P.ng; ++g) {
+    Group& G = P.grp[g];
+    B.kl_tick[g] = mvn_kl_grouped_bwd_slices(G.kl_max_terms_all) > 1
+                       ? sc.get<int>((long long)G.n_prior * mvn_kl_grouped_bwd_blocks(G.M)) : nullptr;
+  }
   sc.get<char>(256);
   const long long z1 = (sc.off + 255) & ~255LL;
   if (!dry) GPSA_CK(zero_fill_async(sc.base + z0, (size_t)(z1 - z0), st));
@@ -1806,9 +1837,13 @@
       const long long mk = sc.mark();
       double* S = sc.get<double>((long long)G.n_prior * mm);
       double* T1 = sc.get<double>((long long)G.n_prior * mm);
-      GPSA_RUN(gpsa_mvn_kl_grouped_bwd_acc(c.mats(G, 0), c.inv(G, 0), G.om_idx, G.pr_list, G.grp_off, G.order,
-                                           c.sv<double>(G.o_D), c.sv<double>(G.o_KD), og.dkl + G.kl_off, G.M, G.n_omega,
-                                           G.n_prior, B.dstack[g] + (long long)G.n_prior * mm, B.dD[g], S, 1, c.stv()));
+      const int ns = mvn_kl_grouped_bwd_slices(G.kl_max_terms), ns_all = mvn_kl_grouped_bwd_slices(G.kl_max_terms_all);
+      double* part = ns_all > 1 ? sc.get<double>((long long)G.n_prior * ns_all * mm) : nullptr;
+      double* gsum = ns_all > 1 ? sc.get<double>((long long)G.n_prior * ns_all * mvn_kl_grouped_bwd_blocks(G.M)) : nullptr;
+      GPSA_RUN(mvn_kl_grouped_bwd_sliced(c.mats(G, 0), c.inv(G, 0), G.om_idx, G.pr_list, G.grp_off, G.order,
+                                         c.sv<double>(G.o_D), c.sv<double>(G.o_KD), og.dkl + G.kl_off, G.M, G.n_omega,
+                                         G.n_prior, B.dstack[g] + (long long)G.n_prior * mm, B.dD[g], S, 1, ns, part,
+                                         gsum, B.kl_tick[g], c.st));
       GPSA_CK(gemm64(c, 0, 0, G.M, G.M, G.M, 1.0, c.inv(G, 0), G.M, mm, S, G.M, mm, 0.0, T1, G.M, mm, G.n_prior,
                      splitk_few(G.M, G.M, G.M, G.n_prior)));
       GPSA_CK(gemm64(c, 0, 0, G.M, G.M, G.M, 0.5, T1, G.M, mm, c.inv(G, 0), G.M, mm, 1.0, B.dstack[g], G.M, mm, G.n_prior,
@@ -1818,7 +1853,19 @@
     return 0;
   };
   auto priors_backward = [&]() -> int {
-    {
+    if (priors_one_launch(P)) {
+      const Run& r = P.runs[0];
+      const long long mk = sc.mark();
+      const long long wsb = gpsa_kmat_bwd_batched_workspace(Mx, Mx, D, r.cnt + 1);
+      void* ws = sc.get<char>(wsb);
+      GPSA_RUN(gpsa_kmat_uu_bwd_batched_tail(
+          P.d.kind_warp, prm.Xtilde + (long long)r.v0 * Mx * D, (long long)Mx * D, Mx, D, prm.warp_ls + r.v0,
+          prm.warp_var + r.v0, 1, r.cnt, prm.Gtilde, prm.data_ls, prm.data_var,
+          B.dstack[0] + (long long)P.pos_Kw(r.b0) * Mx * Mx, (long long)Mx * Mx,
+          B.dstack[P.merged ? 0 : 1] + (long long)P.pos_KF() * Mg * Mg, B.dZ_wu + (long long)r.b0 * Mx * D,
+          (long long)Mx * D, B.dpar_wu + (long long)r.b0 * 2, B.dZ_du, B.dpar_du, ws, wsb, c.stv()));
+      sc.release(mk);
+    } else {
       for (const Run& r : P.runs) {
         const long long mk = sc.mark();
         const long long wsb = gpsa_kmat_bwd_batched_workspace(Mx, Mx, D, r.cnt);
diff --git a/spatial_alignment_amd/ops.py b/spatial_alignment_amd/ops.py
--- a/spatial_alignment_amd/ops.py
+++ b/spatial_alignment_amd/ops.py
@@ -621,6 +621,25 @@
         _lib.check(rc, "gpsa_mvn_kl_grouped_bwd")
         return dOm, dD, S
 
+    def mvn_kl_grouped_bwd_sliced(self, mats, inv, plan, D, KD, g, dOmega=None, sliced=True):
+        T, M = D.shape
+        dev = D.device
+        acc = dOmega is not None
+        dOm = dOmega if acc else torch.empty(T, M, M, dtype=torch.float64, device=dev)
+        dD = torch.empty(T, M, dtype=torch.float64, device=dev)
+        S = torch.empty(plan.P, M, M, dtype=torch.float64, device=dev)
+        off = plan.grp_off.tolist()
+        max_terms = max(off[q + 1] - off[q] for q in range(plan.P)) if sliced else 1
+        tick = torch.zeros(plan.P * ((M * M + 255) // 256), dtype=torch.int32, device=dev)
+        nws = self.lib.gpsa_mvn_kl_grouped_bwd_sliced_workspace(M, plan.P, max_terms)
+        ws = torch.empty(max(nws, 8), dtype=torch.uint8, device=dev)
+        rc = self.lib.gpsa_mvn_kl_grouped_bwd_sliced(_p(mats), _p(inv), _p(plan.om_idx), _p(plan.pr_list),
+                                                     _p(plan.grp_off), _p(plan.order), _p(D), _p(KD), _p(g), M, T,
+                                                     plan.P, _p(dOm), _p(dD), _p(S), int(acc), max_terms, _p(ws), nws,
+                                                     _p(tick), tick.numel(), self._stream(D))
+        _lib.check(rc, "gpsa_mvn_kl_grouped_bwd_sliced")
+        return dOm, dD, S, tick
+
     def elbo_fwd(self, ll, kl, kl_scale):
         ll, kl = self._c(ll), self._c(kl)
         loss = torch.empty(1, dtype=torch.float32, device=ll.device)
```
